# tim-speed/flexdiffuse

Hardware: AMD Instinct MI355X
Metric: 512x512 50-step images/sec/node (SD1.5, batch=8/GPU, Linear image guidance) (higher is better)
Workload: dtype fp16; 1 GPU; SD1.5 512x512 50-step DDIM + linear image guidance, CFG 8, batch=8/GPU (BASELINE configs[1]); parallelism=seed-sharded x1, preset=sd15, guidance=linear, img2img=False, unet_evaluations_per_image=50, launch=graph, scheduler=ddim

## Files before the change

### flexdiffuse_amd/csrc/common.h

```cpp
#pragma once
#include <hip/hip_runtime.h>
#include <stdint.h>
#include <stdio.h>
#include <string.h>

#include "../../include/flexdiffuse_hip.h"

void fd_set_error(const char* fmt, ...);

#define FD_CHECK_ARG(cond, code, ...)                  \
    do {                                               \
        if (!(cond)) {                                 \
            fd_set_error(__VA_ARGS__);                 \
            return (code);                             \
        }                                              \
    } while (0)

#define FD_CHECK_LAUNCH(name)                                                    \
    do {                                                                         \
        hipError_t e_ = hipGetLastError();                                       \
        if (e_ != hipSuccess) {                                                  \
            fd_set_error("%s: launch failed: %s", (name), hipGetErrorString(e_)); \
            return FD_EHIP;                                                      \
        }                                                                        \
    } while (0)

#define FD_HIP(call)                                                                 \
    do {                                                                             \
        hipError_t e_ = (call);                                                      \
        if (e_ != hipSuccess) {                                                      \
            fd_set_error("%s failed: %s", #call, hipGetErrorString(e_));             \
            return FD_EHIP;                                                          \
        }                                                                            \
    } while (0)

static inline int fd_cdiv(int a, int b) { return (a + b - 1) / b; }
static inline int fd_grid1d(size_t total, int cap) {
    const size_t blocks = (total + 255) / 256;
    return (int)(blocks < (size_t)cap ? blocks : (size_t)cap);
}

#ifdef __cplusplus
#include <functional>
bool fd_plan_recording();
void fd_plan_push(std::function<int(void*)> op);
#define FD_PLAN(...)                                                            \
    do {                                                                        \
        if (fd_plan_recording())                                                \
            fd_plan_push([=](void* fd_s_) -> int { return __VA_ARGS__; });      \
    } while (0)
#endif

void fd_prof_begin(int family, hipStream_t s, double work, double executed = -1.0, unsigned tag = 0);
void fd_prof_end(int family, hipStream_t s);
#ifdef __cplusplus
struct FdProfScope {
    int family;
    hipStream_t st;
    FdProfScope(int f, void* stream, double bytes, unsigned tag = 0) : family(f), st((hipStream_t)stream) { fd_prof_begin(f, st, bytes, -1.0, tag); }
    ~FdProfScope() { fd_prof_end(family, st); }
};
static inline unsigned fd_tag(unsigned a, unsigned b = 0, unsigned c = 0, unsigned d = 0, unsigned e = 0, unsigned f = 0) {
    unsigned h = 2166136261u;
    const unsigned v[6] = {a, b, c, d, e, f};
    for (int i = 0; i < 6; ++i) h = (h ^ v[i]) * 16777619u;
    return h | 1u;
}
#endif

#ifdef __cplusplus
#include <atomic>
static inline bool fd_first_on_device(std::atomic<unsigned long long>* mask) {
    int dev = 0;
    if (hipGetDevice(&dev) != hipSuccess) return true;
    const unsigned long long bit = 1ull << (dev & 63);
    return (mask->fetch_or(bit) & bit) == 0;
}
#endif

typedef _Float16 half_t;
typedef half_t half8 __attribute__((ext_vector_type(8)));
typedef half_t half4 __attribute__((ext_vector_type(4)));
typedef half_t half2v __attribute__((ext_vector_type(2)));
typedef float floatx2 __attribute__((ext_vector_type(2)));
typedef float floatx4 __attribute__((ext_vector_type(4)));
typedef float floatx16 __attribute__((ext_vector_type(16)));

__device__ __forceinline__ float fd_wave_sum(float v) {
#pragma unroll
    for (int o = 32; o > 0; o >>= 1) v += __shfl_xor(v, o, 64);
    return v;
}
__device__ __forceinline__ float fd_wave_max(float v) {
#pragma unroll
    for (int o = 32; o > 0; o >>= 1) v = fmaxf(v, __shfl_xor(v, o, 64));
    return v;
}
```

### flexdiffuse_amd/csrc/gemm.hip

```cpp
#include "gemm_epilogue.h"
#include "gn_slab.h"

typedef const __attribute__((address_space(1))) half_t* gptr_h;
typedef const __attribute__((address_space(1))) u32x4* gptr_u4;

template <int BM, int BN, bool TRANS, bool CONV>
__global__ __launch_bounds__(256) void k_gemm_f16(GemmArgs g) {
    constexpr int WTM = BM / 2, WTN = BN / 2;
    constexpr int MI = WTM / 16, NI = WTN / 16;
    constexpr int AR = BM / 32, BR = BN / 32;
    constexpr int STAGE = (BM + BN) * 128;
    extern __shared__ __attribute__((aligned(16))) char smem[];

    const int tid = threadIdx.x, lane = tid & 63, wave = tid >> 6;
    const int wm = wave >> 1, wn = wave & 1;

    const int nb = g.tiles_m * g.tiles_n;
    int id = blockIdx.x;
    {
        const int q = nb >> 3, r = nb & 7, xcd = id & 7, slot = id >> 3;
        id = (xcd < r ? xcd * (q + 1) : r * (q + 1) + (xcd - r) * q) + slot;
    }
    const int tile_n = id % g.tiles_n, tile_m = id / g.tiles_n;
    const int m0 = tile_m * BM, n0 = tile_n * BN;
// ... 694 lines not shown

template <int S>
__device__ __forceinline__ void splitk_finish_body(const GemmArgs& g) {
    const int n4 = g.N >> 2;
    const size_t total = (size_t)g.M * n4;
    const size_t slab = (size_t)g.M * g.N;
    for (size_t e = (size_t)blockIdx.x * 256 + threadIdx.x; e < total; e += (size_t)gridDim.x * 256) {
        const int m = (int)(e / n4), nb0 = (int)(e - (size_t)m * n4) * 4;
        const float* src = g.ws + (size_t)m * g.N + nb0;
        float4 p[S > 0 ? S : 1];
        if constexpr (S > 0) {
#pragma unroll
            for (int s = 0; s < S; ++s) p[s] = *reinterpret_cast<const float4*>(src + (size_t)s * slab);
        } else {
            p[0] = *reinterpret_cast<const float4*>(src);
        }
        float4 bb = make_float4(0.f, 0.f, 0.f, 0.f), b2 = bb;
        half4 rr = {(half_t)0.f, (half_t)0.f, (half_t)0.f, (half_t)0.f};
        if (g.bias) bb = *reinterpret_cast<const float4*>(g.bias + nb0);
        if (g.bias2) b2 = *reinterpret_cast<const float4*>(g.bias2 + (size_t)(m / g.rows_per_batch) * g.ldb2 + nb0);
        if (g.res) rr = *reinterpret_cast<const half4*>(g.res + (size_t)(g.res_rows ? m % g.res_rows : m) * g.ldr + nb0);
        float4 a = p[0];
        if constexpr (S > 0) {
#pragma unroll
            for (int s = 1; s < S; ++s) { a.x += p[s].x; a.y += p[s].y; a.z += p[s].z; a.w += p[s].w; }
        } else {
            for (int s = 1; s < g.split_k; ++s) {
                const float4 q = *reinterpret_cast<const float4*>(src + (size_t)s * slab);
                a.x += q.x; a.y += q.y; a.z += q.z; a.w += q.w;
            }
        }
        const float bs[4] = {bb.x + b2.x, bb.y + b2.y, bb.z + b2.z, bb.w + b2.w};
        float v[4] = {fmaf(a.x, g.alpha, bs[0]), fmaf(a.y, g.alpha, bs[1]), fmaf(a.z, g.alpha, bs[2]), fmaf(a.w, g.alpha, bs[3])};
#pragma unroll
        for (int r = 0; r < 4; ++r) v[r] = act_apply(v[r], g.act);
        if (g.res) {
#pragma unroll
            for (int r = 0; r < 4; ++r) v[r] += (float)rr[r];
        }
        if (g.out_f32) {
            *reinterpret_cast<float4*>(reinterpret_cast<float*>(g.C) + (size_t)m * g.ldc + nb0) =
                make_float4(v[0], v[1], v[2], v[3]);
        } else {
            half4 o;
#pragma unroll
            for (int r = 0; r < 4; ++r) o[r] = (half_t)v[r];
            *reinterpret_cast<half4*>(reinterpret_cast<half_t*>(g.C) + (size_t)m * g.ldc + nb0) = o;
        }
    }
}

__global__ __launch_bounds__(256) void k_splitk_finish(GemmArgs g) {
    switch (g.split_k) {
        case 2: splitk_finish_body<2>(g); break;
        case 4: splitk_finish_body<4>(g); break;
        case 8: splitk_finish_body<8>(g); break;
        case 16: splitk_finish_body<16>(g); break;
        default: splitk_finish_body<0>(g); break;
    }
}


template <int S>
__global__ __launch_bounds__(256) void k_splitk_finish_gn(GemmArgs g) {
    extern __shared__ float gn_sm[];
    constexpr int NT = 256, NV = 16;
    const int HW = g.rows_per_batch, C = g.N, cpg = C / g.gn_groups, GB = g.gn_gb, CB = cpg * GB, c8 = CB >> 3;
    const int b = blockIdx.x, ch0 = blockIdx.y * CB, tid = threadIdx.x;
    const int cc = tid % c8;
    const int n = ch0 + cc * 8;
    float bs[8];
#pragma unroll
    for (int k = 0; k < 8; ++k) bs[k] = 0.f;
    if (g.bias) {
        const float4 lo = *reinterpret_cast<const float4*>(g.bias + n), hi = *reinterpret_cast<const float4*>(g.bias + n + 4);
        bs[0] = lo.x; bs[1] = lo.y; bs[2] = lo.z; bs[3] = lo.w; bs[4] = hi.x; bs[5] = hi.y; bs[6] = hi.z; bs[7] = hi.w;
    }
    if (g.bias2) {
        const float* b2 = g.bias2 + (size_t)b * g.ldb2 + n;
        const float4 lo = *reinterpret_cast<const float4*>(b2), hi = *reinterpret_cast<const float4*>(b2 + 4);
        bs[0] += lo.x; bs[1] += lo.y; bs[2] += lo.z; bs[3] += lo.w; bs[4] += hi.x; bs[5] += hi.y; bs[6] += hi.z; bs[7] += hi.w;
    }
    const size_t slab = (size_t)g.M * g.N;
    const size_t row0 = (size_t)b * HW;
    const float* __restrict__ src0 = g.ws + row0 * g.N + n;
    const int PL = NT / c8, pl = tid / c8;
    const int nv = (HW + PL - 1) / PL;
    const bool active = pl < PL;
    constexpr int CH = S >= 16 ? 1 : (S >= 8 ? 2 : (S >= 4 ? 4 : 8));
    static_assert(NV % CH == 0, "whole chunks");
    auto fill = [&](uint4(&v)[NV]) __attribute__((always_inline)) {
#pragma unroll
        for (int i0 = 0; i0 < NV; i0 += CH) {
            if (i0 < nv) {
                float4 lo[CH][S], hi[CH][S];
                half8 rr[CH];
#pragma unroll
                for (int j = 0; j < CH; ++j) {
                    const int p = min(pl + PL * (i0 + j), HW - 1);
                    const float* src = src0 + (size_t)p * g.N;
#pragma unroll
                    for (int s = 0; s < S; ++s) {
                        lo[j][s] = *reinterpret_cast<const float4*>(src + (size_t)s * slab);
                        hi[j][s] = *reinterpret_cast<const float4*>(src + (size_t)s * slab + 4);
                    }
                }
                if (g.res) {
#pragma unroll
                    for (int j = 0; j < CH; ++j)
                        rr[j] = *reinterpret_cast<const half8*>(g.res + (row0 + min(pl + PL * (i0 + j), HW - 1)) * g.ldr + n);
                }
#pragma unroll
                for (int j = 0; j < CH; ++j) {
                    float a[8] = {lo[j][0].x, lo[j][0].y, lo[j][0].z, lo[j][0].w, hi[j][0].x, hi[j][0].y, hi[j][0].z, hi[j][0].w};
#pragma unroll
                    for (int s = 1; s < S; ++s) {
                        a[0] += lo[j][s].x; a[1] += lo[j][s].y; a[2] += lo[j][s].z; a[3] += lo[j][s].w;
                        a[4] += hi[j][s].x; a[5] += hi[j][s].y; a[6] += hi[j][s].z; a[7] += hi[j][s].w;
                    }
                    half8 o;
#pragma unroll
                    for (int k = 0; k < 8; ++k) {
                        float val = fmaf(a[k], g.alpha, bs[k]);
                        if (g.res) val += (float)rr[j][k];
                        o[k] = (half_t)val;
                    }
                    const int p = pl + PL * (i0 + j);
                    const bool valid = active && p < HW;
                    const uint4 packed = *reinterpret_cast<uint4*>(&o);
                    v[i0 + j] = valid ? packed : make_uint4(0u, 0u, 0u, 0u);
                }
            } else {
#pragma unroll
                for (int j = 0; j < CH; ++j) v[i0 + j] = make_uint4(0u, 0u, 0u, 0u);
            }
        }
        if (!g.gn_skip_c && active) {
            half_t* __restrict__ cb = reinterpret_cast<half_t*>(g.C) + row0 * g.ldc + n;
#pragma unroll
            for (int i = 0; i < NV; ++i) {
                const int p = pl + PL * i;
                if (p < HW) *reinterpret_cast<uint4*>(cb + (size_t)p * g.ldc) = v[i];
            }
        }
    };
    gn_slab_body<NT, NV>(fill, g.gn_out + row0 * C + ch0, g.gn_gamma + ch0, g.gn_beta + ch0, HW, C, cpg, GB, g.gn_eps, g.gn_silu, gn_sm);
}

template <int S>
static int launch_finish_gn(const GemmArgs& g, hipStream_t st) {
    size_t lds = 0;
    const int GB = gn_slab_pick<256, 16>(g.rows_per_batch, g.N, g.gn_groups, &lds);
    static std::atomic<unsigned long long> configured{0};
    if (lds > 64 * 1024 && fd_first_on_device(&configured))
        FD_HIP(hipFuncSetAttribute(reinterpret_cast<const void*>(k_splitk_finish_gn<S>), hipFuncAttributeMaxDynamicSharedMemorySize, 160 * 1024));
    hipLaunchKernelGGL(k_splitk_finish_gn<S>, dim3(g.M / g.rows_per_batch, g.gn_groups / GB), dim3(256), lds, st, g);
    FD_CHECK_LAUNCH("k_splitk_finish_gn");
    return FD_OK;
}

extern "C" int fd_gemm_can_fuse_groupnorm(int M, int N, int rows_per_sample, int groups, int split_k) {
    if (M <= 0 || N <= 0 || rows_per_sample <= 0 || groups <= 0 || M % rows_per_sample != 0 || N % 8 != 0 || N % groups != 0) return 0;
    if (!(split_k == 2 || split_k == 4 || split_k == 8 || split_k == 16)) return 0;
    size_t lds = 0;
    return gn_slab_pick<256, 16>(rows_per_sample, N, groups, &lds) > 0 ? 1 : 0;
}

static bool g_use_dma = getenv("FD_GEMM_NO_DMA") == nullptr;
static int g_tap_fast = getenv("FD_CONV_TAPFAST") ? atoi(getenv("FD_CONV_TAPFAST")) : 1;
static int g_pp = getenv("FD_GEMM_PP") ? atoi(getenv("FD_GEMM_PP")) : 1;
static int g_bias_lds = getenv("FD_GEMM_BIAS_LDS") ? atoi(getenv("FD_GEMM_BIAS_LDS")) : 1;
static int g_fast_epi = getenv("FD_GEMM_FAST_EPI") ? atoi(getenv("FD_GEMM_FAST_EPI")) : 1;
static int g_persist_mode = getenv("FD_GEMM_PERSIST") ? atoi(getenv("FD_GEMM_PERSIST")) : 1;

static bool gemm_lean_dma_path() { return g_use_dma && g_fast_epi && g_bias_lds; }

struct GemmExtents {
    unsigned long long a, w, c;
    static bool below_2gib(unsigned long long elems) { return 2 * elems < 0x7fffffffull; }
    bool dma_ok() const { return below_2gib(a) && below_2gib(w); }
};
static GemmExtents gemm_extents(const GemmArgs& g, bool conv) {
    const unsigned long long a = conv ? ((unsigned long long)(g.M / (g.Ho * g.Wo)) * g.Hi * g.Wi - 1) * g.Cpix + g.Cin : (unsigned long long)(g.M - 1) * g.lda + g.K;
    return {a, (unsigned long long)(g.N - 1) * g.ldw + g.K, (unsigned long long)(g.M - 1) * g.ldc + g.N};
}

template <int BM, int BN, bool TRANS, bool CONV, int WM = 2, int NS = 2, int WN = 2, int EPI = 0>
static int launch_mode(GemmArgs& g, int batch, hipStream_t st) {
    g.tiles_m = fd_cdiv(g.M, BM);
    g.tiles_n = fd_cdiv(g.N, BN);
    const size_t lds = NS * (size_t)(BM + BN) * 128 + 4 * BN * sizeof(float) + ((EPI == 5 || EPI == 6 || EPI == 7 || EPI == 13 || EPI == 14) ? BM * 2 * sizeof(float) : 0);
    dim3 grid(g.tiles_m * g.tiles_n, g.split_k, batch);
    const unsigned long long a_bytes =
        CONV ? 2ull * (((unsigned long long)(g.M / (g.Ho * g.Wo)) * g.Hi * g.Wi - 1) * g.Cpix + g.Cin)
             : 2ull * ((unsigned long long)(g.M - 1) * g.lda + g.K);
    const unsigned long long w_bytes = 2ull * ((unsigned long long)(g.N - 1) * g.ldw + g.K + g.K2);
    if (g_use_dma && a_bytes < 0x7fffffffull && w_bytes < 0x7fffffffull) {
        static std::atomic<unsigned long long> configured{0};
        if (lds > 64 * 1024 && fd_first_on_device(&configured)) {
            FD_HIP(hipFuncSetAttribute(reinterpret_cast<const void*>(k_gemm_f16_dma<BM, BN, CONV, WM, TRANS, NS, WN, EPI>),
                                       hipFuncAttributeMaxDynamicSharedMemorySize, (int)lds));
            if constexpr (BN != 320 && EPI != 13 && EPI != 14)
                FD_HIP(hipFuncSetAttribute(reinterpret_cast<const void*>(k_gemm_f16_dmap<BM, BN, CONV, WM, TRANS, WN, EPI>),
                                           hipFuncAttributeMaxDynamicSharedMemorySize, (int)lds));
        }
        const int occ = (BM >= 256 || lds > 80 * 1024) ? 1 : (BM * BN >= 128 * 128) ? 2 : (BM == 128 ? 3 : 4);
        const int slots = 256 * occ;
        const int nkt = (g.K + BK - 1) / BK / g.split_k;
        const bool persistent = NS == 2 && BN != 320 && EPI != 13 && g.K2 == 0 && !g.phase && !g.ln_stats_out && g.ln_parts <= 1 && g.strideBias == 0 && (g_persist_mode == 2 ||
                                (g_persist_mode == 1 && nkt <= 20 && g.tiles_m * g.tiles_n > slots));
        if constexpr (EPI >= 1 && EPI <= 3) {
            if (persistent && g.bias2) return launch_mode<BM, BN, TRANS, CONV, WM, NS, WN, 0>(g, batch, st);
        }
        if (persistent) {
            if constexpr (BN != 320 && EPI != 13 && EPI != 14) {
                dim3 pgrid(g.tiles_m * g.tiles_n > slots ? slots : g.tiles_m * g.tiles_n, g.split_k, batch);
                hipLaunchKernelGGL((k_gemm_f16_dmap<BM, BN, CONV, WM, TRANS, WN, EPI>), pgrid, dim3(64 * WM * WN), lds,
                                   st, g, (unsigned)a_bytes, (unsigned)w_bytes);
            }
        } else {
            hipLaunchKernelGGL((k_gemm_f16_dma<BM, BN, CONV, WM, TRANS, NS, WN, EPI>), grid, dim3(64 * WM * WN), lds, st, g,
                               (unsigned)a_bytes, (unsigned)w_bytes);
        }
        FD_CHECK_LAUNCH("k_gemm_f16_dma");
        return FD_OK;
    }
    if (g.ln_stats) {
        fd_set_error("fd_gemm_f16: the LayerNorm fold needs the LDS-DMA path (tensor < 2 GiB, FD_GEMM_NO_DMA unset)");
        return FD_ESHAPE;
    }
    if (g.K2) {
        fd_set_error("fd_gemm_f16: the appended 1x1 phase (A2 / K2) needs the LDS-DMA path (tensor < 2 GiB, FD_GEMM_NO_DMA unset)");
        return FD_ESHAPE;
    }
    if constexpr (EPI != 0) {
        return launch_mode<BM, BN, TRANS, CONV, WM, NS, WN, 0>(g, batch, st);
    } else if constexpr (WM != 2 || WN != 2) {
        fd_set_error("fd_gemm_f16: 8-wave tiles need the LDS-DMA path (tensor < 2 GiB)");
        return FD_ESHAPE;
    } else {
        static std::atomic<unsigned long long> configured{0};
        if (lds > 64 * 1024 && fd_first_on_device(&configured))
            FD_HIP(hipFuncSetAttribute(reinterpret_cast<const void*>(k_gemm_f16<BM, BN, TRANS, CONV>),
                                       hipFuncAttributeMaxDynamicSharedMemorySize, (int)lds));
        hipLaunchKernelGGL((k_gemm_f16<BM, BN, TRANS, CONV>), grid, dim3(256), lds, st, g);
        FD_CHECK_LAUNCH("k_gemm_f16");
        return FD_OK;
    }
}

template <int BM, int BN, bool TRANS, int WM = 2, int NS = 2, int WN = 2, int EPI = 0>
static int launch(GemmArgs& g, int batch, hipStream_t st) {
    return g.mode == MODE_CONV ? launch_mode<BM, BN, TRANS, true, WM, NS, WN, EPI>(g, batch, st)
                               : launch_mode<BM, BN, TRANS, false, WM, NS, WN, EPI>(g, batch, st);
}

template <int BM, int BN, int WM, int NS, int WN, int ALLOW>
static int launch_epi(GemmArgs& g, int batch, hipStream_t st) {
    const bool full = g_fast_epi && g.split_k == 1 && !g.out_f32 && !g.trans_out && g.bias_lds &&
                      g.M % BM == 0 && g.N % BN == 0 && (g.ldc & 7) == 0 &&
                      (!g.bias2 || g.rows_per_batch % BM == 0);
    if (g.gn_part_out) {
        if constexpr (BN == 320 && NS == 2) {
            if (full && g.act == FD_ACT_NONE && !g.ln_stats && !g.ln_stats_out && g.N == BN && g.rows_per_batch % BM == 0 && !g.phase && batch == 1 &&
                (!g.res || (g.ldr & 3) == 0)) {
                if (g.res) return launch<BM, BN, false, WM, NS, WN, 12>(g, batch, st);
                return launch<BM, BN, false, WM, NS, WN, 11>(g, batch, st);
            }
        }
        fd_set_error("fd_gemm_f16: gn_part_out needs full 320-wide tiles inside one sample and the lean plain / residual epilogue");
        return FD_ESHAPE;
    }
    if (g.ln_stats_out) {
        if constexpr ((ALLOW & 256) != 0) {
            if (full && (BN != 320 || g.N == BN) && g.act == FD_ACT_NONE && g.mode != MODE_CONV && !g.ln_stats && !g.bias2) {
                if (g.res && (g.ldr & 3) == 0) return launch_mode<BM, BN, false, false, WM, NS, WN, 9>(g, batch, st);
                if (!g.res) return launch_mode<BM, BN, false, false, WM, NS, WN, 8>(g, batch, st);
            }
        }
        fd_set_error("fd_gemm_f16: ln_stats_out needs full tiles of a tile shape with a statistics epilogue, a plain or residual linear GEMM");
        return FD_ESHAPE;
    }
    if (full && g.ln_stats) {
        if (g.mode != MODE_CONV && !g.res) {
            if constexpr ((ALLOW & 64) != 0 && (BN / WN / 16) % 2 == 0) {
                if (g.act == FD_ACT_GEGLU) return launch_mode<BM, BN, false, false, WM, NS, WN, 6>(g, batch, st);
            }
            if constexpr ((ALLOW & 32) != 0) {
                if (g.act == FD_ACT_NONE) return launch_mode<BM, BN, false, false, WM, NS, WN, 5>(g, batch, st);
            }
        }
        return launch_mode<128, 128, false, false, 2, 2, 2, 7>(g, batch, st);
    }
    if (g.ln_stats) return launch_mode<128, 128, false, false, 2, 2, 2, 7>(g, batch, st);
    if (full) {
        if constexpr ((ALLOW & 8) != 0 && (BN / WN / 16) % 2 == 0) {
            if (g.act == FD_ACT_GEGLU) return launch<BM, BN, false, WM, NS, WN, 3>(g, batch, st);
        }
        if constexpr ((ALLOW & 4) != 0) {
            if (g.act == FD_ACT_NONE && g.res && (g.ldr & 3) == 0) return launch<BM, BN, false, WM, NS, WN, 2>(g, batch, st);
        }
        if constexpr ((ALLOW & 2) != 0) {
            if (g.act == FD_ACT_NONE && !g.res) return launch<BM, BN, false, WM, NS, WN, 1>(g, batch, st);
        }
    }
    return launch<BM, BN, false, WM, NS, WN, 0>(g, batch, st);
}

#include "gemm_xfold.h"

static double fd_round_eff(long long tiles, int slots) {
    return (double)tiles / (double)((long long)slots * ((tiles + slots - 1) / slots));
}

static int fd_stats_plan(int M, int N, int* tile, int batch = 1) {
    if (N < 320 || N % 160 != 0) return 0;
    const bool ok23 = M % 288 == 0 && M >= 1152;
    if (N == 320 && M % 256 == 0) {
        if (ok23 && fd_round_eff((long long)(M / 288) * 2, 256) > fd_round_eff(M / 256, 256) + 0.08) {
            *tile = 23;
            return 2;
        }
        *tile = 16;
        return 1;
    }
    if (ok23 && (M % 128 != 0 ||
                 fd_round_eff((long long)(M / 288) * (N / 160), 256) >
                     (M % 256 == 0 && M > 4096 ? fd_round_eff((long long)(M / 256) * (N / 160), 256)
                                                : fd_round_eff((long long)(M / 128) * (N / 160), 512)) + 0.08)) {
        *tile = 23;
        return N / 160;
    }
    if (N != 320 && batch > 1 && M % 64 == 0 && M % 128 != 0) {
        *tile = 26;
        return N / 160;
    }
    if (N == 320 || M % 128 != 0) return 0;
    if (batch > 1 && M <= 256 && N >= 1280) {
        *tile = 20;
        return N / 160;
    }
    *tile = (M % 256 == 0 && (long long)M * batch > 4096) ? 13 : 12;
    return N / 160;
}

extern "C" int fd_gemm_can_emit_row_stats(int M, int N, int K, int ldc, int ldr) {
    if (!gemm_lean_dma_path()) return 0;
    if (M <= 0 || K <= 0 || K % 8 != 0) return 0;
    if (ldc < N || (ldc & 7) != 0 || (ldr != 0 && (ldr < N || (ldr & 3) != 0))) return 0;
    if (!GemmExtents::below_2gib((unsigned long long)(M - 1) * (unsigned long long)ldc + N)) return 0;
    int tile = 0;
    return fd_stats_plan(M, N, &tile);
}


struct GemmPlan {
    int tile, split, batch;
    int gn_parts_bm;
    double flops, flops_exec;
    unsigned tag;
};

enum { FORM_RULE, FORM_TRANS_TAIL, FORM_SOFTMAX, FORM_TRANS_OUT };
static int gemm_form(const GemmArgs& g) { return g.tr_n0 ? FORM_TRANS_TAIL : (g.sm_valid ? FORM_SOFTMAX : (g.trans_out ? FORM_TRANS_OUT : FORM_RULE)); }

static void gemm_tile_shape(int tile, int* bm, int* bn) {
    switch (tile) {
        case 9: case 12: case 20: *bm = 128; *bn = 160; break;
        case 10: *bm = 128; *bn = 128; break;
        case 13: *bm = 256; *bn = 160; break;
        case 14: *bm = 256; *bn = 128; break;
        case 15: *bm = 256; *bn = 256; break;
        case 16: *bm = 256; *bn = 320; break;
        case 23: *bm = 288; *bn = 160; break;
        case 26: *bm = 64; *bn = 160; break;
        default: fd_gemm_pp_tile_shape(tile, bm, bn); break;
    }
}

static bool gemm_tile_ln_fold(int tile) {
    return tile == 9 || tile == 10 || (tile >= 12 && tile <= 16) || tile == 20 || tile == 23 || tile == 26 || tile >= 30;
}

static bool gemm_pp_ok(GemmArgs g, int batch, int tile, int split) {
    g.split_k = split;
    return fd_gemm_pp_ok(g, batch, tile);
}

static int gemm_grow_split(const GemmArgs& g, size_t ws_bytes, long long tiles, int target, int cap, int min_kt) {
    if (!g.ws || g.N % 4 != 0) return 1;
    const int nk_all = (g.K + g.K2 + BK - 1) / BK;
    int split = 1;
    while (tiles * split < target && split < cap && nk_all / (split * 2) >= min_kt && (size_t)(split * 2) * g.M * g.N * 4 <= ws_bytes) split *= 2;
    return split;
}

static int gn_parts_bm(const GemmArgs& g, int tile, int split, int batch, int groups) {
// ... 448 lines not shown
```

### flexdiffuse_amd/csrc/gemm_pp.hip

```cpp
#include "gemm_epilogue.h"

typedef __attribute__((address_space(3))) void* lds_ptr;

template <int WM_, int WN_, int MI, int NI, bool CONV, int EPI, bool HAS_K2>
__global__ __launch_bounds__(512) void k_gemm_f16_pp(GemmArgs g, unsigned a_bytes, unsigned w_bytes) {
#if defined(__HIP_DEVICE_COMPILE__)
    static_assert(WM_ * WN_ == 8 && MI % 2 == 0, "8 waves; the row halves must be equal");
    constexpr int WTM = MI * 16, WTN = NI * 16, BM = WM_ * WTM, BN = WN_ * WTN;
    constexpr int MH = MI / 2, NI0 = (NI + 1) / 2, NI1 = NI / 2;
    constexpr int PA = WM_ * MH * 16, PB0 = WN_ * NI0 * 16, PB1 = WN_ * NI1 * 16;
    constexpr int OA0 = 0, OB0 = PA * 128, OB1 = OB0 + PB0 * 128, OA1 = OB1 + PB1 * 128, STAGE = OA1 + PA * 128;
    constexpr int GA = PA / 8, GB0 = PB0 / 8, GB1 = PB1 / 8;
    constexpr int CA = (GA + 7) / 8, CB0 = (GB0 + 7) / 8, CB1 = (GB1 + 7) / 8;
    static_assert(GA % 8 == 0 && GB1 % 8 == 0, "only B0 may leave some waves one DMA short");
    constexpr int INFLIGHT = 2 * (GA / 8) + GB0 / 8 + GB1 / 8;
    extern __shared__ __attribute__((aligned(16))) char smem[];

#ifdef FD_PP_STAMPS
    const unsigned long long ts_start = __builtin_amdgcn_s_memtime();
    const unsigned long long rt_start = __builtin_amdgcn_s_memrealtime();
    unsigned long long ts_a[4] = {0, 0, 0, 0}, ts_b[4] = {0, 0, 0, 0}, ts_d[4] = {0, 0, 0, 0};
#define PP_STAMP(X) X = __builtin_amdgcn_s_memtime();
#else
#define PP_STAMP(X)
// ... 249 lines not shown
    PP_BAR();
    const bool late = wave >= 4;
    if (late) { PP_BAR(); }
#ifdef FD_PP_STAMPS
    const unsigned long long ts_loop0 = __builtin_amdgcn_s_memtime();
#endif
    int l = 0;
#pragma clang loop unroll(disable)
    for (; l + 1 < nkl; l += 2) {
        PP_PHASE(0) PP_PHASE(1) PP_PHASE(2) PP_PHASE(3)
        PP_PHASE(4) PP_PHASE(5) PP_PHASE(6) PP_PHASE(7)
    }
#ifdef FD_PP_STAMPS
    const unsigned long long ts_sa[4] = {ts_a[0], ts_a[1], ts_a[2], ts_a[3]}, ts_sb[4] = {ts_b[0], ts_b[1], ts_b[2], ts_b[3]},
                             ts_sd[4] = {ts_d[0], ts_d[1], ts_d[2], ts_d[3]};
#endif
    if (l < nkl) {
        PP_PHASE(0) PP_PHASE(1) PP_PHASE(2) PP_PHASE(3)
    }
    if (!late) { PP_BAR(); }
#ifdef FD_PP_STAMPS
    const unsigned long long ts_loop1 = __builtin_amdgcn_s_memtime();
#endif
#undef PP_PHASE
#undef PP_WAIT
#undef PP_BAR
#undef PP_MFMA
#undef PP_READ_A
#undef PP_READ_B0
#undef PP_READ_B1
#undef PP_ISSUE
#undef PP_ISSUE_A
#undef PP_ISSUE_B
#undef PP_PREP
#undef PP_PREP_A
#undef PP_PREP_B
#undef PP_ADVANCE
#undef PP_GROUP_ROW
#undef PP_B_ROW
#undef PP_IS_A2
#undef PP_UNIFORM
#undef PP_FLAG

    if constexpr (EPI == 10) {
        float* __restrict__ P = g.ws + (size_t)kslice * g.M * g.N + (size_t)(m0 + wm * WTM + fr) * g.N + n0 + wn * WTN + fq * 4;
#pragma unroll
        for (int i = 0; i < MI; ++i)
#pragma unroll
            for (int j = 0; j < NI; ++j) {
#ifdef FD_SPLITK_NO_STORE
                asm volatile("" ::"v"(acc[i][j]));
                if (g.M < 0)
#endif
                *reinterpret_cast<floatx4*>(P + (size_t)i * 16 * g.N + j * 16) = acc[i][j];
            }
    } else if constexpr (EPI == 14) {
        {
            float* __restrict__ P = g.ws + (size_t)kslice * g.M * g.N + (size_t)(m0 + wm * WTM + fr) * g.N + n0 + wn * WTN + fq * 4;
#pragma unroll
            for (int i = 0; i < MI; ++i)
#pragma unroll
                for (int j = 0; j < NI; ++j) *reinterpret_cast<floatx4*>(P + (size_t)i * 16 * g.N + j * 16) = acc[i][j];
        }
        const int tile_id = tile_m * g.tiles_n + tile_n;
        unsigned* arrive = g.sk_sync + tile_id;
        unsigned* depart = g.sk_sync + g.tiles_m * g.tiles_n + tile_id;
        __syncthreads();
        if (tid == 0) {
            __hip_atomic_fetch_add(arrive, 1u, __ATOMIC_RELEASE, __HIP_MEMORY_SCOPE_AGENT);
            int spins = 0;
            while (__hip_atomic_load(arrive, __ATOMIC_ACQUIRE, __HIP_MEMORY_SCOPE_AGENT) < (unsigned)g.split_k && ++spins < (1 << 22))
                __builtin_amdgcn_s_sleep(4);
        }
        __syncthreads();
        {
            const int S = g.split_k, rows = BM / S, r0 = m0 + kslice * rows;
            constexpr int C4 = BN / 4;
            const size_t slab = (size_t)g.M * g.N;
            for (int e = tid; e < rows * C4; e += 512) {
                const int r = e / C4, c4 = e - r * C4;
                const int m = r0 + r, n = n0 + c4 * 4;
                const float* src = g.ws + (size_t)m * g.N + n;
                float4 a = *reinterpret_cast<const float4*>(src);
                for (int sidx = 1; sidx < S; ++sidx) {
                    const float4 q = *reinterpret_cast<const float4*>(src + (size_t)sidx * slab);
                    a.x += q.x; a.y += q.y; a.z += q.z; a.w += q.w;
                }
                float4 bb = make_float4(0.f, 0.f, 0.f, 0.f), b2 = bb;
                if (g.bias) bb = *reinterpret_cast<const float4*>(g.bias + n);
                if (g.bias2) b2 = *reinterpret_cast<const float4*>(g.bias2 + (size_t)(m / g.rows_per_batch) * g.ldb2 + n);
                float v[4] = {fmaf(a.x, g.alpha, bb.x + b2.x), fmaf(a.y, g.alpha, bb.y + b2.y), fmaf(a.z, g.alpha, bb.z + b2.z), fmaf(a.w, g.alpha, bb.w + b2.w)};
                if (g.res) {
                    const half4 rr = *reinterpret_cast<const half4*>(g.res + (size_t)(g.res_rows ? m % g.res_rows : m) * g.ldr + n);
#pragma unroll
                    for (int k = 0; k < 4; ++k) v[k] += (float)rr[k];
                }
                half4 o;
#pragma unroll
                for (int k = 0; k < 4; ++k) o[k] = (half_t)v[k];
                *reinterpret_cast<half4*>(reinterpret_cast<half_t*>(g.C) + (size_t)m * g.ldc + n) = o;
            }
        }
        __syncthreads();
        if (tid == 0) {
            const unsigned old = __hip_atomic_fetch_add(depart, 1u, __ATOMIC_RELAXED, __HIP_MEMORY_SCOPE_AGENT);
            if (old == (unsigned)g.split_k - 1u) {
                __hip_atomic_store(arrive, 0u, __ATOMIC_RELAXED, __HIP_MEMORY_SCOPE_AGENT);
                __hip_atomic_store(depart, 0u, __ATOMIC_RELAXED, __HIP_MEMORY_SCOPE_AGENT);
            }
        }
    } else if constexpr (EPI == 0 || EPI == 7)
        gemm_epilogue<BM, BN, false, WM_, WN_, EPI == 7>(g, acc, m0, n0, wm, wn, fr, fq, z, (g.bias && g.bias_lds) ? (lds_cfloat)bias_s : (lds_cfloat) nullptr,
                                                         b2_staged ? (lds_cfloat)(bias_s + BN) : (lds_cfloat) nullptr, kslice, stats_tile);
    else if constexpr (EPI == 8 || EPI == 9) {
        asm volatile("s_waitcnt vmcnt(0)" ::: "memory");
        __syncthreads();
        gemm_epilogue_fast<MI, NI, FD_ACT_NONE, EPI == 9, true, false, true, WN_>(
            g, acc, m0 + wm * WTM + fr, n0 + wn * WTN, wn * WTN, fq, z, (lds_cfloat)bias_s, (lds_cfloat)(bias_s + BN),
            reinterpret_cast<float*>(smem), wm * WTM + fr, wn, m0);
    } else if constexpr (EPI == 11 || EPI == 12) {
        asm volatile("s_waitcnt vmcnt(0)" ::: "memory");
        __syncthreads();
        gemm_epilogue_fast<MI, NI, FD_ACT_NONE, EPI == 12, true, false, false, WN_, WM_>(
            g, acc, m0 + wm * WTM + fr, n0 + wn * WTN, wn * WTN, fq, z, (lds_cfloat)bias_s, (lds_cfloat)(bias_s + BN),
            reinterpret_cast<float*>(smem), wm * WTM + fr, wn, m0);
    } else
        gemm_epilogue_fast<MI, NI, (EPI == 3 || EPI == 6) ? FD_ACT_GEGLU : FD_ACT_NONE, EPI == 2, true, (EPI == 5 || EPI == 6)>(
            g, acc, m0 + wm * WTM + fr, n0 + wn * WTN, wn * WTN, fq, z, (lds_cfloat)bias_s, (lds_cfloat)(bias_s + BN),
            nullptr, wm * WTM + fr, wn, m0, stats_tile);
#ifdef FD_PP_STAMPS
    if (EPI != 10 && g.ws && lane == 0) {
        unsigned long long* o = reinterpret_cast<unsigned long long*>(g.ws) + ((size_t)blockIdx.x * 8 + wave) * 16;
        o[0] = ts_start; o[1] = ts_loop0; o[2] = ts_loop1; o[3] = __builtin_amdgcn_s_memtime();
#pragma unroll
        for (int p = 0; p < 3; ++p) { o[4 + 3 * p] = ts_sa[p]; o[5 + 3 * p] = ts_sb[p]; o[6 + 3 * p] = ts_sd[p]; }
        o[13] = ts_sa[3]; o[14] = ts_sb[3];
        o[15] = __builtin_amdgcn_s_memrealtime() - rt_start;
    }
#endif
#undef PP_STAMP
#endif
}

template <int WM_, int WN_, int MI, int NI, bool CONV, int EPI, bool HAS_K2>
static int pp_launch_k2(GemmArgs& g, int batch, hipStream_t st) {
    constexpr int BM = WM_ * MI * 16, BN = WN_ * NI * 16;
    g.tiles_m = g.M / BM;
    g.tiles_n = g.N / BN;
    const size_t lds = 2 * (size_t)(BM + BN) * 128 + 4 * BN * sizeof(float) + ((EPI == 5 || EPI == 6 || EPI == 7) ? BM * 2 * sizeof(float) : 0);
    const unsigned long long a_bytes = CONV ? 2ull * (((unsigned long long)(g.M / (g.Ho * g.Wo)) * g.Hi * g.Wi - 1) * g.Cpix + g.Cin)
                                            : 2ull * ((unsigned long long)(g.M - 1) * g.lda + g.K);
    const unsigned long long w_bytes = 2ull * ((unsigned long long)(g.N - 1) * g.ldw + g.K + g.K2);
    static std::atomic<unsigned long long> configured{0};
    if (fd_first_on_device(&configured))
        FD_HIP(hipFuncSetAttribute(reinterpret_cast<const void*>(k_gemm_f16_pp<WM_, WN_, MI, NI, CONV, EPI, HAS_K2>),
                                   hipFuncAttributeMaxDynamicSharedMemorySize, (int)lds));
    static const int sk_xcd = getenv("FD_PP_SK_XCD") ? atoi(getenv("FD_PP_SK_XCD")) : 1;
    const int nb = g.tiles_m * g.tiles_n;
    g.sk_flat = sk_xcd && (g.split_k == 2 || g.split_k == 4 || g.split_k == 8) && batch == 1 && nb % (8 / g.split_k) == 0 &&
                (nb * g.split_k) % 8 == 0;
    const dim3 grid = g.sk_flat ? dim3(nb * g.split_k, 1, batch) : dim3(nb, g.split_k, batch);
    hipLaunchKernelGGL((k_gemm_f16_pp<WM_, WN_, MI, NI, CONV, EPI, HAS_K2>), grid, dim3(512), lds, st, g,
                       (unsigned)a_bytes, (unsigned)w_bytes);
    FD_CHECK_LAUNCH("k_gemm_f16_pp");
    return FD_OK;
}

template <int WM_, int WN_, int MI, int NI, bool CONV, int EPI>
static int pp_launch_k(GemmArgs& g, int batch, hipStream_t st) {
    if constexpr (EPI == 1 || EPI == 2 || EPI == 10 || EPI == 0 || EPI == 11 || EPI == 12 || EPI == 14) {
        if (g.K2) return pp_launch_k2<WM_, WN_, MI, NI, CONV, EPI, true>(g, batch, st);
    } else {
        if (g.K2) {
            fd_set_error("fd_gemm_f16: the appended A2 phase has no ping-pong kernel with this epilogue");
            return FD_ESHAPE;
        }
    }
    return pp_launch_k2<WM_, WN_, MI, NI, CONV, EPI, false>(g, batch, st);
}

template <int WM_, int WN_, int MI, int NI>
static int pp_launch(GemmArgs& g, int batch, hipStream_t st) {
    constexpr int BM = WM_ * MI * 16, BN = WN_ * NI * 16;
    const bool conv = g.mode == MODE_CONV;
    if (g.split_k > 1 && (g.N & 3) == 0 && g.sk_sync) {
        if constexpr (BN == 320) {
            if ((g.M / BM) * (g.N / BN) * g.split_k <= 256 && BM % g.split_k == 0 && batch == 1 && !g.out_f32 && g.act == FD_ACT_NONE && (g.ldc & 3) == 0 &&
                (!g.res || (g.ldr & 3) == 0) && (g.ldb2 & 3) == 0)
                return conv ? pp_launch_k<WM_, WN_, MI, NI, true, 14>(g, batch, st) : pp_launch_k<WM_, WN_, MI, NI, false, 14>(g, batch, st);
        }
        fd_set_error("fd_gemm_f16: sk_sync (in-launch split-K reduction) needs a 320-wide ping-pong tile, tiles x split_k <= 256 workgroups, a plain fp16 output");
        return FD_ESHAPE;
    }
    if (g.split_k > 1 && (g.N & 3) == 0)
        return conv ? pp_launch_k<WM_, WN_, MI, NI, true, 10>(g, batch, st) : pp_launch_k<WM_, WN_, MI, NI, false, 10>(g, batch, st);
    const bool lean = g.split_k == 1 && !g.out_f32 && !g.trans_out && g.bias_lds && (g.ldc & 7) == 0 &&
                      (!g.bias2 || g.ln_stats || g.rows_per_batch % BM == 0);
    if (g.gn_part_out) {
        if constexpr (BN == 320) {
            if (lean && g.act == FD_ACT_NONE && !g.ln_stats && !g.ln_stats_out && g.N == BN && g.rows_per_batch % BM == 0 && !g.phase && batch == 1 &&
                (!g.res || (g.ldr & 3) == 0)) {
                if (g.res) return conv ? pp_launch_k<WM_, WN_, MI, NI, true, 12>(g, batch, st) : pp_launch_k<WM_, WN_, MI, NI, false, 12>(g, batch, st);
                return conv ? pp_launch_k<WM_, WN_, MI, NI, true, 11>(g, batch, st) : pp_launch_k<WM_, WN_, MI, NI, false, 11>(g, batch, st);
            }
        }
        fd_set_error("fd_gemm_f16: gn_part_out on a ping-pong tile needs the lean epilogue of a 320-wide tile inside one sample");
        return FD_ESHAPE;
    }
    if (g.ln_stats_out) {
        if (lean && !conv && (WN_ == 2 || g.N == BN) && g.act == FD_ACT_NONE && !g.ln_stats && !g.bias2) {
            if (g.res && (g.ldr & 3) == 0) return pp_launch_k<WM_, WN_, MI, NI, false, 9>(g, batch, st);
            if (!g.res) return pp_launch_k<WM_, WN_, MI, NI, false, 8>(g, batch, st);
        }
        fd_set_error("fd_gemm_f16: ln_stats_out on a ping-pong tile needs the lean epilogue of a plain or residual linear GEMM");
        return FD_ESHAPE;
    }
    if (g.ln_stats) {
        if (lean && !conv && !g.res) {
            if constexpr (NI % 2 == 0) {
                if (g.act == FD_ACT_GEGLU) return pp_launch_k<WM_, WN_, MI, NI, false, 6>(g, batch, st);
            }
            if (g.act == FD_ACT_NONE) return pp_launch_k<WM_, WN_, MI, NI, false, 5>(g, batch, st);
        }
        if (!conv) return pp_launch_k<WM_, WN_, MI, NI, false, 7>(g, batch, st);
        fd_set_error("fd_gemm_f16: LayerNorm fold on a convolution");
        return FD_ESHAPE;
    }
    if (lean) {
        if constexpr (NI % 2 == 0) {
            if (g.act == FD_ACT_GEGLU && !conv) return pp_launch_k<WM_, WN_, MI, NI, false, 3>(g, batch, st);
        }
        if (g.act == FD_ACT_NONE && g.res && (g.ldr & 3) == 0)
            return conv ? pp_launch_k<WM_, WN_, MI, NI, true, 2>(g, batch, st) : pp_launch_k<WM_, WN_, MI, NI, false, 2>(g, batch, st);
        if (g.act == FD_ACT_NONE && !g.res)
            return conv ? pp_launch_k<WM_, WN_, MI, NI, true, 1>(g, batch, st) : pp_launch_k<WM_, WN_, MI, NI, false, 1>(g, batch, st);
    }
    return conv ? pp_launch_k<WM_, WN_, MI, NI, true, 0>(g, batch, st) : pp_launch_k<WM_, WN_, MI, NI, false, 0>(g, batch, st);
}

void fd_gemm_pp_tile_shape(int tile, int* bm, int* bn) {
    switch (tile) {
        case 30: *bm = 256; *bn = 320; break;
        case 31: *bm = 256; *bn = 256; break;
        case 32: *bm = 128; *bn = 320; break;
        case 33: *bm = 256; *bn = 160; break;
        default: *bm = *bn = 0; break;
    }
}

bool fd_gemm_pp_ok(const GemmArgs& g, int batch, int tile) {
    int bm, bn;
    fd_gemm_pp_tile_shape(tile, &bm, &bn);
    if (!bm) return false;
    if (g.M % bm != 0 || g.N % bn != 0 || g.K % BK != 0 || g.K2 % BK != 0 || g.trans_out) return false;
    if (g.act == FD_ACT_GEGLU && (bn / (tile == 33 ? 2 : 4)) % 32 != 0) return false;
    const unsigned long long a_bytes = g.mode == MODE_CONV ? 2ull * (((unsigned long long)(g.M / (g.Ho * g.Wo)) * g.Hi * g.Wi - 1) * g.Cpix + g.Cin)
                                                           : 2ull * ((unsigned long long)(g.M - 1) * g.lda + g.K);
    const unsigned long long w_bytes = 2ull * ((unsigned long long)(g.N - 1) * g.ldw + g.K + g.K2);
    if (a_bytes >= 0x7ffffff0ull || w_bytes >= 0x7ffffff0ull) return false;
    if (g.mode == MODE_CONV) {
        if (g.Wo % 8 != 0 || g.up || g.Cin % BK != 0) return false;
        if (g.K2 && (g.stride != 1 || g.Ho != g.Hi || g.Wo != g.Wi || g.phase)) return false;
    }
    if (g.split_k > 1 && (g.K / BK + g.K2 / BK) / g.split_k < 2) return false;
    (void)batch;
    return true;
}

int fd_gemm_pp_launch(GemmArgs& g, int batch, hipStream_t st, int tile) {
    switch (tile) {
        case 30: return pp_launch<2, 4, 8, 5>(g, batch, st);
        case 31: return pp_launch<2, 4, 8, 4>(g, batch, st);
        case 32: return pp_launch<2, 4, 4, 5>(g, batch, st);
        case 33: return pp_launch<4, 2, 4, 5>(g, batch, st);
        default: fd_set_error("fd_gemm_f16: unknown ping-pong tile %d", tile); return FD_EINVAL;
    }
}
```

### flexdiffuse_amd/csrc/norm.hip

```cpp
#include <stdlib.h>

#include "common.h"
#include "gn_slab.h"

#define GN_MAX_CHUNKS 256

__global__ void k_gn_stats(const half_t* __restrict__ x, float* __restrict__ part, int HW, int C,
                           int G, int PL, int pix_per_chunk, int ldx) {
    extern __shared__ float sm[];
    const int b = blockIdx.y, chunk = blockIdx.x;
    const int c8 = C >> 3;
    const int tid = threadIdx.x;
    const int cc = tid % c8, pl = tid / c8;
    const int p0 = chunk * pix_per_chunk;
    const int p1 = min(HW, p0 + pix_per_chunk);
    float s[8], q[8];
#pragma unroll
    for (int k = 0; k < 8; ++k) s[k] = q[k] = 0.f;
    if (pl < PL) {
        const half_t* base = x + ((size_t)b * HW) * ldx + cc * 8;
        int p = p0 + pl;
        uint4 raw[4], nxt[4];
        bool have = p + 3 * PL < p1;
        if (have) {
// ... 59 lines not shown
            bq += sm[(size_t)(g * cpg + i) * 2 + 1];
        }
        a = fd_wave_sum(a);
        bq = fd_wave_sum(bq);
        if (lane == 0) {
            float* dst = part + (((size_t)b * gridDim.x + chunk) * G + g) * 2;
            dst[0] = a;
            dst[1] = bq;
        }
    }
}

__global__ void k_gn_apply(const half_t* __restrict__ x, half_t* __restrict__ y,
                           const float* __restrict__ part, const float* __restrict__ gamma,
                           const float* __restrict__ beta, int HW, int C, int G,
                           int nchunk_stats, int PL, int pix_per_chunk, float eps, int silu, int ldx) {
    extern __shared__ float sm[];
    const int b = blockIdx.y, chunk = blockIdx.x, tid = threadIdx.x;
    const int nt = blockDim.x, nsub = nt / G;
    double* red = reinterpret_cast<double*>(sm);
    float* gst = reinterpret_cast<float*>(red + 2 * nsub * G);
    {
        const int g = tid % G, sub = tid / G;
        if (sub < nsub) {
            double s = 0.0, q = 0.0;
            const float2* src = reinterpret_cast<const float2*>(part) + ((size_t)b * nchunk_stats) * G + g;
            int k = sub;
            for (; k + 3 * nsub < nchunk_stats; k += 4 * nsub) {
                float2 v[4];
#pragma unroll
                for (int u = 0; u < 4; ++u) v[u] = src[(size_t)(k + u * nsub) * G];
#pragma unroll
                for (int u = 0; u < 4; ++u) {
                    s += (double)v[u].x;
                    q += (double)v[u].y;
                }
            }
            for (; k < nchunk_stats; k += nsub) {
                const float2 v = src[(size_t)k * G];
                s += (double)v.x;
                q += (double)v.y;
            }
            red[sub * G + g] = s;
            red[nsub * G + sub * G + g] = q;
        }
    }
    __syncthreads();
    const int cpg = C / G;
    if (tid < G) {
        double s = 0.0, q = 0.0;
        for (int u = 0; u < nsub; ++u) {
            s += red[u * G + tid];
            q += red[nsub * G + u * G + tid];
        }
        const double n = (double)HW * cpg;
        const double mean = s / n;
        double var = q / n - mean * mean;
        if (var < 0.0) var = 0.0;
        gst[tid * 2 + 0] = (float)mean;
        gst[tid * 2 + 1] = (float)(1.0 / sqrt(var + (double)eps));
    }
    __syncthreads();
    const int c8 = C >> 3;
    const int cc = tid % c8, pl = tid / c8;
    if (pl >= PL) return;
    float sc[8], sh[8];
#pragma unroll
    for (int k = 0; k < 8; ++k) {
        const int c = cc * 8 + k, g = c / cpg;
        const float a = gst[g * 2 + 1] * gamma[c];
        sc[k] = a;
        sh[k] = beta[c] - gst[g * 2 + 0] * a;
    }
    const int p0 = chunk * pix_per_chunk;
    const int p1 = min(HW, p0 + pix_per_chunk);
    const half_t* xb = x + ((size_t)b * HW) * ldx + cc * 8;
    half_t* yb = y + ((size_t)b * HW) * C + cc * 8;
    int p = p0 + pl;
    uint4 raw[4], nxt[4];
    bool have = p + 3 * PL < p1;
    if (have) {
#pragma unroll
        for (int u = 0; u < 4; ++u) raw[u] = *reinterpret_cast<const uint4*>(xb + (size_t)(p + u * PL) * ldx);
    }
    while (have) {
        const int pn = p + 4 * PL;
        const bool more = pn + 3 * PL < p1;
        if (more) {
#pragma unroll
            for (int u = 0; u < 4; ++u) nxt[u] = *reinterpret_cast<const uint4*>(xb + (size_t)(pn + u * PL) * ldx);
        }
#pragma unroll
        for (int u = 0; u < 4; ++u) {
            const half8 v = *reinterpret_cast<const half8*>(&raw[u]);
            half8 o;
#pragma unroll
            for (int k = 0; k < 8; ++k) o[k] = (half_t)gn_act(fmaf((float)v[k], sc[k], sh[k]), silu);
            *reinterpret_cast<uint4*>(yb + (size_t)(p + u * PL) * C) = *reinterpret_cast<uint4*>(&o);
        }
#pragma unroll
        for (int u = 0; u < 4; ++u) raw[u] = nxt[u];
        p = pn;
        have = more;
    }
    for (; p < p1; p += PL) {
        const uint4 raw = *reinterpret_cast<const uint4*>(xb + (size_t)p * ldx);
        const half8 v = *reinterpret_cast<const half8*>(&raw);
        half8 o;
#pragma unroll
        for (int k = 0; k < 8; ++k) o[k] = (half_t)gn_act(fmaf((float)v[k], sc[k], sh[k]), silu);
        *reinterpret_cast<uint4*>(yb + (size_t)p * C) = *reinterpret_cast<uint4*>(&o);
    }
}

template <int NT, int NV>
__global__ __launch_bounds__(NT) void k_gn_slab(const half_t* __restrict__ x, half_t* __restrict__ y,
                                                const float* __restrict__ gamma,
                                                const float* __restrict__ beta, int HW, int C,
                                                int G, int GB, float eps, int silu, int ldx) {
    extern __shared__ float sm[];
    const int cpg = C / G, CB = cpg * GB, c8 = CB >> 3;
    const int PL = NT / c8;
    const int b = blockIdx.x, ch0 = blockIdx.y * CB, tid = threadIdx.x;
    const int cc = tid % c8, pl = tid / c8;
    const half_t* xb = x + (size_t)b * HW * ldx + ch0;
    const unsigned xoff0 = (unsigned)(pl * ldx + cc * 8), xstep = (unsigned)(PL * ldx);
    const bool active = pl < PL;
    gn_slab_body<NT, NV>(
        [&](uint4(&v)[NV]) __attribute__((always_inline)) {
#pragma unroll
            for (int i = 0; i < NV; ++i) {
                const int p = pl + PL * i;
                v[i] = make_uint4(0u, 0u, 0u, 0u);
                if (active && p < HW) v[i] = *reinterpret_cast<const uint4*>(xb + (xoff0 + xstep * i));
            }
        },
        y + (size_t)b * HW * C + ch0, gamma + ch0, beta + ch0, HW, C, cpg, GB, eps, silu, sm);
}

template <int NT, int NV>
static bool gn_try_slab(const void* x, void* y, const float* gamma, const float* beta, int B,
                        int HW, int C, int G, float eps, int silu, hipStream_t st, int* rc, int ldx) {
    size_t lds = 0;
    const int GB = gn_slab_pick<NT, NV>(HW, C, G, &lds);
    if (!GB) return false;
    static std::atomic<unsigned long long> attr_set{0};
    if (fd_first_on_device(&attr_set)) {
        if (hipFuncSetAttribute(reinterpret_cast<const void*>(k_gn_slab<NT, NV>),
                                hipFuncAttributeMaxDynamicSharedMemorySize, 160 * 1024) != hipSuccess) {
            fd_set_error("fd_groupnorm_nhwc_f16: cannot raise the LDS limit");
            *rc = FD_EHIP;
            return true;
        }
    }
    fd_prof_begin(FD_FAMILY_GROUPNORM, st, (double)B * HW * C * 4.0, -1.0, fd_tag(7u, B, HW, C, NT));
    hipLaunchKernelGGL((k_gn_slab<NT, NV>), dim3(B, G / GB), dim3(NT), lds, st, (const half_t*)x,
                       (half_t*)y, gamma, beta, HW, C, G, GB, eps, silu, ldx);
    fd_prof_end(FD_FAMILY_GROUPNORM, st);
    *rc = hipGetLastError() == hipSuccess ? FD_OK : FD_EHIP;
    if (*rc != FD_OK) fd_set_error("k_gn_slab: launch failed");
    return true;
}

#define GNF_ROWS 16
__global__ __launch_bounds__(256) void k_gn_fold_linear(const float* __restrict__ part, int nchunk_stats, int HW, int C, int G, float eps,
                                                        const half_t* __restrict__ wg,
                                                        const float* __restrict__ biasf, int N, half_t* __restrict__ w_out,
                                                        float* __restrict__ bias_out) {
    __shared__ float rstd_s[64], mean_s[64];
    __shared__ float gsum_s[GNF_ROWS][64];
    __shared__ double red_s[2][256];
    extern __shared__ __align__(16) unsigned char gnf_lds[];
    half_t* wr = reinterpret_cast<half_t*>(gnf_lds);
    const int b = blockIdx.y, tid = threadIdx.x;
    const int nsub = 256 / G;
    {
        const int g = tid % G, sub = tid / G;
        if (sub < nsub) {
            double s = 0.0, q = 0.0;
            const float2* src = reinterpret_cast<const float2*>(part) + ((size_t)b * nchunk_stats) * G + g;
            for (int k = sub; k < nchunk_stats; k += nsub) {
                const float2 v = src[(size_t)k * G];
                s += (double)v.x;
                q += (double)v.y;
            }
            red_s[0][sub * G + g] = s;
            red_s[1][sub * G + g] = q;
        }
    }
    __syncthreads();
    if (tid < G) {
        double s = 0.0, q = 0.0;
        for (int u = 0; u < nsub; ++u) {
            s += red_s[0][u * G + tid];
            q += red_s[1][u * G + tid];
        }
        const double n = (double)HW * (C / G);
        const double mean = s / n;
        double var = q / n - mean * mean;
        if (var < 0.0) var = 0.0;
        const double rstd = 1.0 / sqrt(var + (double)eps);
        rstd_s[tid] = (float)rstd;
        mean_s[tid] = (float)mean;
    }
    __syncthreads();
    const int n0 = blockIdx.x * GNF_ROWS, rows = min(GNF_ROWS, N - n0);
    const int c8 = C >> 3, cpg = C / G;
    for (int i = tid; i < rows * c8; i += 256) {
        const int r = i / c8, cc = i - r * c8;
        const half8 v = *reinterpret_cast<const half8*>(wg + (size_t)(n0 + r) * C + cc * 8);
        half8 o;
#pragma unroll
        for (int k = 0; k < 8; ++k) o[k] = (half_t)((float)v[k] * rstd_s[(cc * 8 + k) / cpg]);
        *reinterpret_cast<half8*>(w_out + ((size_t)b * N + n0 + r) * C + cc * 8) = o;
        *reinterpret_cast<half8*>(wr + (size_t)r * C + cc * 8) = o;
    }
    __syncthreads();
    for (int i = tid; i < rows * G; i += 256) {
        const int r = i / G, g = i - r * G;
        const half_t* src = wr + (size_t)r * C + g * cpg;
        float acc = 0.f;
        for (int c = 0; c < cpg; ++c) acc += (float)src[c];
        gsum_s[r][g] = acc;
    }
    __syncthreads();
    if (tid < rows) {
        float acc = biasf[n0 + tid];
        for (int g = 0; g < G; ++g) acc = fmaf(-mean_s[g], gsum_s[tid][g], acc);
        bias_out[(size_t)b * N + n0 + tid] = acc;
    }
}

static void gn_stats_shape(int B, int HW, int C, int* PL, int* threads, int* nchunk, int* ppc) {
    const int c8 = C / 8;
    int pl = 512 / c8;
    if (pl < 1) pl = 1;
    if (pl > HW) pl = HW;
    int nc = 256 / B;
    if (nc < 1) nc = 1;
    if (nc > GN_MAX_CHUNKS) nc = GN_MAX_CHUNKS;
    int pp = fd_cdiv(HW, nc);
    if (pp < pl) pp = pl;
    *PL = pl;
    *threads = ((c8 * pl + 63) / 64) * 64;
    *ppc = pp;
    *nchunk = fd_cdiv(HW, pp);
}

extern "C" int fd_groupnorm_fold_linear_f16(const void* x, int ldx, float* ws, int B, int HW, int C, int G, float eps,
                                            const void* wg, const float* biasf, int N,
                                            void* w_out, float* bias_out, void* stream) {
    FD_PLAN(fd_groupnorm_fold_linear_f16(x, ldx, ws, B, HW, C, G, eps, wg, biasf, N, w_out, bias_out, fd_s_));
    FD_CHECK_ARG(x && ws && wg && biasf && w_out && bias_out, FD_EINVAL, "fd_groupnorm_fold_linear_f16: null pointer");
    FD_CHECK_ARG(B > 0 && HW > 0 && C > 0 && G > 0 && N > 0, FD_EINVAL, "fd_groupnorm_fold_linear_f16: bad dims");
    FD_CHECK_ARG(C % 8 == 0 && C % G == 0 && G <= 64 && C / 8 <= 1024, FD_ESHAPE,
                 "fd_groupnorm_fold_linear_f16: C=%d must be a multiple of 8 and of G=%d (G <= 64)", C, G);
    FD_CHECK_ARG(ldx >= C && ldx % 8 == 0 && ((uintptr_t)x | (uintptr_t)wg | (uintptr_t)w_out) % 16 == 0, FD_ESHAPE,
                 "fd_groupnorm_fold_linear_f16: ldx=%d must be >= C=%d, a multiple of 8; x / wg / w_out 16-byte aligned", ldx, C);
    FD_CHECK_ARG((long long)B * HW * ldx < 0x7fffffffLL, FD_ESHAPE, "fd_groupnorm_fold_linear_f16: tensor too large");
    hipStream_t st = (hipStream_t)stream;
    int PL, threads, nchunk, ppc;
    gn_stats_shape(B, HW, C, &PL, &threads, &nchunk, &ppc);
    const size_t lds1 = (size_t)PL * C * 2 * sizeof(float);
    FD_CHECK_ARG(lds1 <= 64 * 1024, FD_ESHAPE, "fd_groupnorm_fold_linear_f16: stats LDS too large");
    const size_t lds2 = (size_t)GNF_ROWS * C * sizeof(half_t);
    FD_CHECK_ARG(lds2 <= 48 * 1024, FD_ESHAPE, "fd_groupnorm_fold_linear_f16: C=%d too wide for the fold kernel's weight tile", C);
    fd_prof_begin(FD_FAMILY_GROUPNORM, st, (double)B * HW * C * 2.0, -1.0, fd_tag(8u, B, HW, C, N));
    hipLaunchKernelGGL(k_gn_stats, dim3(nchunk, B), dim3(threads), lds1, st, (const half_t*)x, ws, HW, C, G, PL, ppc, ldx);
    hipLaunchKernelGGL(k_gn_fold_linear, dim3(fd_cdiv(N, GNF_ROWS), B), dim3(256), lds2, st, (const float*)ws, nchunk, HW, C, G, eps,
                       (const half_t*)wg, biasf, N, (half_t*)w_out, bias_out);
    fd_prof_end(FD_FAMILY_GROUPNORM, st);
    FD_CHECK_LAUNCH("k_gn_stats/k_gn_fold_linear");
    return FD_OK;
}

extern "C" int fd_groupnorm_fold_linear_parts_f16(const float* parts, int chunks, int B, int HW, int C, int G, float eps,
                                                  const void* wg, const float* biasf, int N, void* w_out, float* bias_out, void* stream) {
    FD_PLAN(fd_groupnorm_fold_linear_parts_f16(parts, chunks, B, HW, C, G, eps, wg, biasf, N, w_out, bias_out, fd_s_));
    FD_CHECK_ARG(parts && wg && biasf && w_out && bias_out, FD_EINVAL, "fd_groupnorm_fold_linear_parts_f16: null pointer");
    FD_CHECK_ARG(B > 0 && HW > 0 && C > 0 && G > 0 && N > 0 && chunks > 0, FD_EINVAL, "fd_groupnorm_fold_linear_parts_f16: bad dims");
    FD_CHECK_ARG(C % 8 == 0 && C % G == 0 && G <= 64 && ((uintptr_t)wg | (uintptr_t)w_out) % 16 == 0, FD_ESHAPE,
                 "fd_groupnorm_fold_linear_parts_f16: C=%d must be a multiple of 8 and of G=%d (G <= 64); wg / w_out 16-byte aligned", C, G);
    const size_t lds2 = (size_t)GNF_ROWS * C * sizeof(half_t);
    FD_CHECK_ARG(lds2 <= 48 * 1024, FD_ESHAPE, "fd_groupnorm_fold_linear_parts_f16: C=%d too wide for the fold kernel's weight tile", C);
    hipStream_t st = (hipStream_t)stream;
    fd_prof_begin(FD_FAMILY_GROUPNORM, st, 0.0, -1.0, fd_tag(12u, B, HW, C, N));
    hipLaunchKernelGGL(k_gn_fold_linear, dim3(fd_cdiv(N, GNF_ROWS), B), dim3(256), lds2, st, parts, chunks, HW, C, G, eps,
                       (const half_t*)wg, biasf, N, (half_t*)w_out, bias_out);
    fd_prof_end(FD_FAMILY_GROUPNORM, st);
    FD_CHECK_LAUNCH("k_gn_fold_linear");
    return FD_OK;
}

extern "C" int64_t fd_groupnorm_workspace_floats(int B, int G) {
    return (int64_t)B * GN_MAX_CHUNKS * G * 2;
}

extern "C" int fd_groupnorm_nhwc_f16(const void* x, void* y, const float* gamma,
                                     const float* beta, float* ws, int B, int HW, int C, int G,
                                     float eps, int silu, void* stream) {
    return fd_groupnorm_nhwc_ld_f16(x, C, y, gamma, beta, ws, B, HW, C, G, eps, silu, stream);
}

extern "C" int fd_groupnorm_nhwc_ld_f16(const void* x, int ldx, void* y, const float* gamma,
                                        const float* beta, float* ws, int B, int HW, int C, int G,
                                        float eps, int silu, void* stream) {
// ... 283 lines not shown
```

### flexdiffuse_amd/csrc/xattn.hip

```cpp
#include <stdlib.h>

#include "common.h"

#define XBK 64
typedef unsigned int xu32x2 __attribute__((ext_vector_type(2)));
typedef unsigned int xu32x4 __attribute__((ext_vector_type(4)));
typedef const __attribute__((address_space(3))) float* xlds_cfloat;
typedef const __attribute__((address_space(3))) floatx4* xlds_cf4;

struct XattnArgs {
    const half_t* A;
    const half_t* W;
    const float* bias;
    const float* colsum;
    const float* ln_stats;
    const char* kimg;
    const char* vimg;
    half_t* O;
    int M, lda, ldw, ldo;
    int rows_per_sample, samples_per_rep, n_keys;
    int ln_parts;
    float ln_inv_n, ln_eps;
};

// ... 222 lines not shown
#pragma unroll
            for (int j = 0; j < NI; ++j) {
                if (j + 1 < NI) fb[j + 1] = *reinterpret_cast<const half8*>(st + frag_b + (j + 1) * 2048 + sw);
#pragma unroll
                for (int i = 0; i < MI; ++i) acc[i][j] = __builtin_amdgcn_mfma_f32_16x16x32_f16(fb[j], fa[i], acc[i][j], 0, 0, 0);
                __builtin_amdgcn_sched_barrier(0);
            }
        }
        asm volatile("s_waitcnt vmcnt(0)" ::: "memory");
        __syncthreads();
        cur ^= 1;
    }
    const char* sK = smem + cur * STAGE;
    const char* sV = smem + (cur ^ 1) * STAGE;
    XA_DMA_IMAGE(rsVi, VIMG, cur ^ 1);

    half8 q0[MI], q1[MI], qT[MI];
    {
        floatx2 st[MI];
#pragma unroll
        for (int i = 0; i < MI; ++i)
            st[i] = *reinterpret_cast<const __attribute__((address_space(3))) floatx2*>(
                (xlds_cfloat)stats_s + 2 * (wm * WTM + i * 16 + fr));
#pragma unroll
        for (int j = 0; j < NI; ++j) {
            const floatx4 bb = *reinterpret_cast<xlds_cf4>((xlds_cfloat)bias_s + wn * WTN + j * 16 + fq * 4);
            const floatx4 cs = *reinterpret_cast<xlds_cf4>((xlds_cfloat)bias_s + BN + wn * WTN + j * 16 + fq * 4);
            constexpr int JT = D == 40 ? 2 : 4;
#pragma unroll
            for (int i = 0; i < MI; ++i)
#pragma unroll
                for (int r = 0; r < 4; ++r) {
                    const half_t q = (half_t)fmaf(acc[i][j][r], st[i][0], fmaf(st[i][1], cs[r], bb[r]));
                    if (j == JT) { qT[i][r] = q; qT[i][4 + r] = (half_t)0.f; }
                    else {
                        const int jj = j < JT ? j : j - 1;
                        if (jj == 0) q0[i][r] = q;
                        if (jj == 1) q0[i][4 + r] = q;
                        if (jj == 2) q1[i][r] = q;
                        if (jj == 3) q1[i][4 + r] = q;
                    }
                }
            __builtin_amdgcn_sched_barrier(0);
        }
    }
    const int kb_last_valid = g.n_keys - 64 - fq * 4;
    const __amdgpu_buffer_rsrc_t rsO = __builtin_amdgcn_make_buffer_rsrc((void*)g.O, 0, o_bytes, 0x00020000);
    const unsigned o_lane = (unsigned)(((m0 + wm * WTM + fr) * g.ldo + n0 + wn * WTN + fq * 4) * 2);
    const unsigned o_rep = (unsigned)rep * (unsigned)g.M * (unsigned)g.ldo * 2u;
    bool v_ready = false;
#pragma unroll
    for (int hh = 0; hh < cfg::HPW; ++hh) {
        const char* kh = sK + (wn * cfg::HPW + hh) * KHEAD;
        const char* vh = sV + (wn * cfg::HPW + hh) * VHEAD;
#pragma unroll
        for (int ip = 0; ip < MI / 2; ++ip) {
            floatx4 s[2][XA_KB];
#pragma unroll
            for (int kb = 0; kb < XA_KB; ++kb) {
                const half8 ka = *reinterpret_cast<const half8*>(kh + kb * KBB + lane * 16);
                half8 kbf = ka;
                if constexpr (D == 80) kbf = *reinterpret_cast<const half8*>(kh + kb * KBB + 1024 + lane * 16);
                const half4 k16 = *reinterpret_cast<const half4*>(kh + kb * KBB + cfg::KSF * 1024 + lane * 8);
                const half_t z = (half_t)0.f;
                const half8 k16x = {k16[0], k16[1], k16[2], k16[3], z, z, z, z};
#pragma unroll
                for (int t = 0; t < 2; ++t) {
                    const int i = ip * 2 + t;
                    floatx4 v;
                    if constexpr (D == 40) {
                        v = __builtin_amdgcn_mfma_f32_16x16x32_f16(ka, hh ? q1[i] : q0[i], floatx4{0.f, 0.f, 0.f, 0.f}, 0, 0, 0);
                    } else {
                        v = __builtin_amdgcn_mfma_f32_16x16x32_f16(ka, q0[i], floatx4{0.f, 0.f, 0.f, 0.f}, 0, 0, 0);
                        v = __builtin_amdgcn_mfma_f32_16x16x32_f16(kbf, q1[i], v, 0, 0, 0);
                    }
                    s[t][kb] = __builtin_amdgcn_mfma_f32_16x16x32_f16(k16x, qT[i], v, 0, 0, 0);
                }
            }
            half8 pk[2][3];
            float lsum[2] = {0.f, 0.f};
#pragma unroll
            for (int t = 0; t < 2; ++t) {
#pragma unroll
                for (int r = 0; r < 4; ++r)
                    if (r >= kb_last_valid) s[t][4][r] = -INFINITY;
                float mx = fmaxf(fmaxf(s[t][0][0], s[t][0][1]), fmaxf(s[t][0][2], s[t][0][3]));
#pragma unroll
                for (int kb = 1; kb < XA_KB; ++kb)
                    mx = fmaxf(mx, fmaxf(fmaxf(s[t][kb][0], s[t][kb][1]), fmaxf(s[t][kb][2], s[t][kb][3])));
                mx = fmaxf(mx, __shfl_xor(mx, 16, 64));
                mx = fmaxf(mx, __shfl_xor(mx, 32, 64));
#pragma unroll
                for (int kb = 0; kb < XA_KB; ++kb)
#pragma unroll
                    for (int r = 0; r < 4; ++r) {
                        const half_t ph = (half_t)__builtin_amdgcn_exp2f(s[t][kb][r] - mx);
                        pk[t][kb >> 1][(kb & 1) * 4 + r] = ph;
                        if constexpr (!cfg::ONES) lsum[t] += (float)ph;
                    }
#pragma unroll
                for (int r = 0; r < 4; ++r) pk[t][2][4 + r] = (half_t)0.f;
                if constexpr (!cfg::ONES) {
                    lsum[t] += __shfl_xor(lsum[t], 16, 64);
                    lsum[t] += __shfl_xor(lsum[t], 32, 64);
                }
            }
            if (!v_ready) {
                asm volatile("s_waitcnt vmcnt(0)" ::: "memory");
                __syncthreads();
                v_ready = true;
            }
            floatx4 o[2][cfg::DT];
#pragma unroll
            for (int dt = 0; dt < cfg::DT; ++dt) {
                const half8 v0 = *reinterpret_cast<const half8*>(vh + dt * 2560 + lane * 16);
                const half8 v1 = *reinterpret_cast<const half8*>(vh + dt * 2560 + 1024 + lane * 16);
                const half4 v2 = *reinterpret_cast<const half4*>(vh + dt * 2560 + 2048 + lane * 8);
                const half_t z = (half_t)0.f;
                const half8 v2x = {v2[0], v2[1], v2[2], v2[3], z, z, z, z};
#pragma unroll
                for (int t = 0; t < 2; ++t) {
                    floatx4 a = __builtin_amdgcn_mfma_f32_16x16x32_f16(v0, pk[t][0], floatx4{0.f, 0.f, 0.f, 0.f}, 0, 0, 0);
                    a = __builtin_amdgcn_mfma_f32_16x16x32_f16(v1, pk[t][1], a, 0, 0, 0);
                    o[t][dt] = __builtin_amdgcn_mfma_f32_16x16x32_f16(v2x, pk[t][2], a, 0, 0, 0);
                }
            }
#pragma unroll
            for (int t = 0; t < 2; ++t) {
                float l = lsum[t];
                if constexpr (cfg::ONES) l = __shfl(o[t][2][0], 32 + fr, 64);
                const float inv = __builtin_amdgcn_rcpf(l);
                const unsigned off = o_lane + (unsigned)(((ip * 2 + t) * 16 * g.ldo + hh * D) * 2);
#pragma unroll
                for (int dt = 0; dt < cfg::DT; ++dt) {
                    half4 v;
#pragma unroll
                    for (int r = 0; r < 4; ++r) v[r] = (half_t)(o[t][dt][r] * inv);
                    const unsigned vo = (D == 40 && dt == 2 && fq >= 2) ? 0xffffff00u : off + dt * 32;
                    __builtin_amdgcn_raw_buffer_store_b64(__builtin_bit_cast(xu32x2, v), rsO, vo, o_rep, 0);
                }
            }
        }
    }
#undef XA_DMA_TILE
#undef XA_DMA_IMAGE
#endif
}

template <int D>
static int xa_launch(const XattnArgs& g, int n_rep, unsigned a_bytes, unsigned w_bytes, unsigned o_bytes, hipStream_t st) {
    typedef XaCfg<D> cfg;
    constexpr size_t lds = 2 * (size_t)(cfg::BM + 320) * 128 + (2 * 320 + 2 * cfg::BM) * sizeof(float);
    static std::atomic<unsigned long long> configured{0};
    if (fd_first_on_device(&configured))
        FD_HIP(hipFuncSetAttribute(reinterpret_cast<const void*>(k_xattn<D>), hipFuncAttributeMaxDynamicSharedMemorySize, (int)lds));
    hipLaunchKernelGGL(k_xattn<D>, dim3(g.M / cfg::BM, n_rep, cfg::C / 320), dim3(1024), lds, st, g, a_bytes, w_bytes, o_bytes);
    return FD_OK;
}

extern "C" int fd_xattn_q_f16(const fd_xattn_desc* d, void* stream) {
    if (fd_plan_recording() && d) {
        const fd_xattn_desc dc_ = *d;
        fd_plan_push([dc_](void* fd_s_) -> int { return fd_xattn_q_f16(&dc_, fd_s_); });
    }
    FD_CHECK_ARG(d && d->x && d->wq && d->bias && d->ln_colsum && d->ln_stats && d->k_image && d->v_image && d->out,
                 FD_EINVAL, "fd_xattn_q_f16: null pointer");
    FD_CHECK_ARG(xa_supported(d->heads, d->head_dim), FD_ESHAPE,
                 "fd_xattn_q_f16: 8 heads x 40 or 8 x 80 only (got %d x %d)", d->heads, d->head_dim);
    const int C = d->heads * d->head_dim, bm = d->head_dim == 40 ? 256 : 128;
    FD_CHECK_ARG(d->M > 0 && d->M % bm == 0 && d->rows_per_sample > 0 && d->rows_per_sample % bm == 0 &&
                     d->M % d->rows_per_sample == 0,
                 FD_ESHAPE, "fd_xattn_q_f16: M=%d and rows_per_sample=%d must be multiples of %d", d->M, d->rows_per_sample, bm);
    FD_CHECK_ARG(d->n_keys > 64 && d->n_keys <= 80 && d->n_rep >= 1, FD_ESHAPE, "fd_xattn_q_f16: 65..80 keys, n_rep >= 1 (got %d keys)", d->n_keys);
    FD_CHECK_ARG(d->ldx % 8 == 0 && d->ldw % 8 == 0 && d->ldo % 4 == 0 && d->ldx >= C && d->ldw >= C && d->ldo >= C,
                 FD_ESHAPE, "fd_xattn_q_f16: leading dimensions");
    FD_CHECK_ARG((((uintptr_t)d->x | (uintptr_t)d->wq | (uintptr_t)d->k_image | (uintptr_t)d->v_image | (uintptr_t)d->bias |
                   (uintptr_t)d->ln_colsum | (uintptr_t)d->ln_stats) % 16 == 0) && (uintptr_t)d->out % 8 == 0,
                 FD_ESHAPE, "fd_xattn_q_f16: pointers must be 16-byte aligned");
    const unsigned long long a_bytes = 2ull * ((unsigned long long)(d->M - 1) * d->ldx + C);
    const unsigned long long w_bytes = 2ull * ((unsigned long long)(C - 1) * d->ldw + C);
    const unsigned long long o_bytes = 2ull * ((unsigned long long)((long long)d->n_rep * d->M - 1) * d->ldo + C);
    FD_CHECK_ARG(a_bytes < 0x7fffffffull && o_bytes < 0x7fffffffull, FD_ESHAPE, "fd_xattn_q_f16: tensor >= 2 GiB");
    XattnArgs g;
    g.A = (const half_t*)d->x; g.W = (const half_t*)d->wq; g.bias = d->bias; g.colsum = d->ln_colsum;
    g.ln_stats = d->ln_stats; g.kimg = (const char*)d->k_image; g.vimg = (const char*)d->v_image;
    g.O = (half_t*)d->out;
    g.M = d->M; g.lda = d->ldx; g.ldw = d->ldw; g.ldo = d->ldo;
    g.rows_per_sample = d->rows_per_sample;
    g.samples_per_rep = d->M / d->rows_per_sample; g.n_keys = d->n_keys;
    FD_CHECK_ARG(d->ln_stats_parts == 0 || d->ln_stats_parts == 2 || d->ln_stats_parts == 4 || d->ln_stats_parts == 8, FD_ESHAPE,
                 "fd_xattn_q_f16: ln_stats_parts=%d (0, 2, 4 or 8)", d->ln_stats_parts);
    g.ln_parts = d->ln_stats_parts; g.ln_inv_n = 1.0f / (float)C; g.ln_eps = d->ln_fold_eps > 0.f ? d->ln_fold_eps : 1e-5f;
    hipStream_t st = (hipStream_t)stream;
    const double flops = 2.0 * d->M * (double)C * C + 4.0 * (double)d->n_rep * d->M * d->n_keys * C;
    fd_prof_begin(FD_FAMILY_ATTENTION, st, flops, -1.0, fd_tag(5u, d->M, d->n_rep, d->head_dim, d->n_keys));
    const int rc = d->head_dim == 40 ? xa_launch<40>(g, d->n_rep, (unsigned)a_bytes, (unsigned)w_bytes, (unsigned)o_bytes, st)
                                     : xa_launch<80>(g, d->n_rep, (unsigned)a_bytes, (unsigned)w_bytes, (unsigned)o_bytes, st);
    fd_prof_end(FD_FAMILY_ATTENTION, st);
    if (rc != FD_OK) return rc;
    FD_CHECK_LAUNCH("k_xattn");
    return FD_OK;
}
```

### flexdiffuse_amd/hip.py

```python
from __future__ import annotations

import ctypes
import os
from ctypes import c_char_p, c_double, c_float, c_int, c_int32, c_int64, c_uint64, c_void_p
from typing import Optional

import torch

_HERE = os.path.dirname(os.path.abspath(__file__))
LIB_PATH = os.environ.get('FD_LIB_PATH') or os.path.join(_HERE, 'libflexdiffuse_hip.so')

FD_OK, FD_EINVAL, FD_ESHAPE, FD_EHIP = 0, -1, -2, -3


class FDError(RuntimeError):
    '''HIP runtime failure reported by libflexdiffuse_hip.so (FD_EHIP).'''


class fd_tween_params(ctypes.Structure):
    _fields_ = [('threshold_floor', c_double), ('threshold_mult', c_double),
                ('clustered', c_double), ('max_guidance', c_double),
                ('header_max', c_double), ('order', c_int32), ('reuse', c_int32)]


P = c_void_p
_SIGNATURES = {
    'fd_abi_version': (c_int, []),
    'fd_last_error': (c_char_p, []),
    'fd_device_info': (c_int, [c_int, P, P, P, P, c_int]),
    'fd_prof_enable': (c_int, [c_int]),
    'fd_prof_set_stride': (c_int, [c_int]),
    'fd_prof_collect': (c_int, [c_int, P, P, P]),
    'fd_prof_collect2': (c_int, [c_int, P, P, P, P]),
    'fd_prof_calibrate': (c_int, [c_int, P, P]),
    'fd_prof_drain': (c_int, [P, P, P, P, P, c_int64, P]),
    'fd_guidance_workspace_floats': (c_int64, [c_int, c_int, c_int]),
    'fd_guidance_map': (c_int, [P, P, P, P, P, c_int, c_int, c_int, c_int, c_int, c_int, c_int, P]),
    'fd_guidance_tween': (c_int, [P, P, P, P, P, P, P, P, P, c_int, c_int, c_int, c_int, c_int,
                                  ctypes.POINTER(fd_tween_params), P]),
    'fd_guidance_concept_override': (c_int, [P, P, P, P, P, c_int, c_int, c_int, P]),
    'fd_guidance_header_pull': (c_int, [P, P, c_int, c_int, c_int, P]),
    'fd_gemm_f16': (c_int, [P, P]),
    'fd_gemm_can_emit_row_stats': (c_int, [c_int, c_int, c_int, c_int, c_int]),
    'fd_gemm_plan': (c_int, [c_void_p, c_void_p, c_void_p]),
    'fd_gemm_can_fuse_groupnorm': (c_int, [c_int, c_int, c_int, c_int, c_int]),
    'fd_gemm_gn_parts_chunks': (c_int, [P]),
    'fd_groupnorm_apply_parts_f16': (c_int, [P, c_int, P, P, P, P, c_int, c_int, c_int, c_int, c_int, c_float, c_int, P]),
    'fd_groupnorm_fold_linear_parts_f16': (c_int, [P, c_int, c_int, c_int, c_int, c_int, c_float, P, P, c_int, P, P, P]),
    'fd_attention_f16': (c_int, [P, P]),
    'fd_xattn_image_bytes': (c_int64, [c_int, c_int]),
    'fd_xattn_pack_kv_f16': (c_int, [P, P, P, P, c_int, c_int, c_int, c_int, c_int, c_int, c_int64, c_int64, P]),
    'fd_xattn_q_f16': (c_int, [P, P]),
    'fd_groupnorm_workspace_floats': (c_int64, [c_int, c_int]),
    'fd_groupnorm_nhwc_f16': (c_int, [P, P, P, P, P, c_int, c_int, c_int, c_int, c_float, c_int, P]),
    'fd_groupnorm_nhwc_ld_f16': (c_int, [P, c_int, P, P, P, P, c_int, c_int, c_int, c_int, c_float, c_int, P]),
    'fd_layernorm_f16': (c_int, [P, P, P, P, c_int, c_int, c_int, c_int, c_float, c_int, P]),
    'fd_ln_row_stats_f16': (c_int, [P, P, c_int, c_int, c_int, c_float, P]),
    'fd_ln_finalize_stats_f32': (c_int, [P, P, c_int, c_int, c_int, c_float, P]),
    'fd_groupnorm_fold_linear_f16': (c_int, [P, c_int, P, c_int, c_int, c_int, c_int, c_float, P, P, c_int, P, P, P]),
    'fd_softmax_rows_f16': (c_int, [P, c_int, c_int, c_int, c_float, P]),
    'fd_nchw_f32_to_nhwc_f16': (c_int, [P, P, c_int, c_int, c_int, c_int, c_int, c_float, P]),
    'fd_nhwc_f32_to_nchw_f32': (c_int, [P, P, c_int, c_int, c_int, c_int, c_float, c_float, c_int, P]),
    'fd_im2col_f16': (c_int, [P, P] + [c_int] * 12 + [P]),
    'fd_conv3x3_narrow_f16': (c_int, [P, P, P, P, c_int, P, c_int, c_int, c_int, c_int, c_int, c_int, c_int, c_float, P]),
    'fd_concat_channels_f16': (c_int, [P, P, P, c_int64, c_int, c_int, P]),
    'fd_cfg_ddim_step_f32': (c_int, [P, P, P, c_int, c_int, c_int, c_int, c_int, c_float, c_float,
                                     c_float, c_float, c_float, c_int, c_int, P]),
    'fd_axpby_f32': (c_int, [P, P, P, c_int64, c_float, c_float, c_int, P]),
    'fd_embed_tokens_f16': (c_int, [P, P, P, P, c_int, c_int, c_int, c_int, P]),
    'fd_vit_assemble_f16': (c_int, [P, P, P, P, c_int, c_int, c_int, P]),
    'fd_timestep_embedding_f16': (c_int, [P, c_int, P, c_int, c_int, P]),
    'fd_copy2d_f16': (c_int, [P, c_int, P, c_int, c_int64, c_int, P]),
    'fd_repeat_rows_f16': (c_int, [P, c_int, P, c_int, c_int64, c_int, c_int, P]),
    'fd_plan_create': (c_int, [P]),
    'fd_plan_destroy': (c_int, [P]),
    'fd_plan_record_begin': (c_int, [P]),
    'fd_plan_record_end': (c_int, [P]),
    'fd_plan_size': (c_int, [P, P]),
    'fd_plan_replay': (c_int, [P, P]),
    'fd_region_blend_f32': (c_int, [P, P] + [c_int] * 7 + [c_float, P]),
    'fd_composite_step_f32': (c_int, [P, P, P, P, c_int, c_int, c_int, c_int, c_int, c_int, c_float, c_float,
                                      c_float, c_float, c_float, c_int, c_int, P]),
    'fd_cfg_ddim_masked_step_f32': (c_int, [P, P, P, P, P, c_int, c_int, c_int, c_int, c_int, c_float, c_float,
                                            c_float, c_float, c_float, c_int, c_float, c_float, P]),
    'fd_cfg_multistep_step_f32': (c_int, [P, P, P, P, P, P, P, c_int, c_int, c_int, c_int, c_int, c_float, c_float,
                                          c_float, c_float, c_float, c_float, c_float, c_float, P]),
    'fd_cfg_linear_multistep_step_f32': (c_int, [P, P, c_int, c_int] + [P] * 10 + [c_int] * 5 + [c_float] * 11 + [P]),
    'fd_philox_normal_f32': (c_int, [P, c_int64, c_int, c_uint64, c_int64, c_int, c_int, P]),
    'fd_cfg_ddim_noise_step_f32': (c_int, [P, P, P, P, P, c_int, c_int, c_int, c_int, c_int, c_float, c_float,
                                           c_float, c_float, c_float, c_int, c_float, c_float, c_float, c_uint64, c_int64,
                                           c_int, c_int, P]),
    'fd_cfg_multistep_noise_step_f32': (c_int, [P, P, P, P, P, P, P, c_int, c_int, c_int, c_int, c_int, c_float, c_float,
                                                c_float, c_float, c_float, c_float, c_float, c_float, c_float, c_uint64,
                                                c_int64, c_int, c_int, P]),
    'fd_cfg_rescale_ddim_step_f32': (c_int, [P, P, P, P, P, P, P, c_int, c_int, c_int, c_int, c_float, c_float, c_float,
                                             c_float, c_float, c_float, c_int, c_int, c_float, c_float, c_float, c_uint64,
                                             c_int64, c_int, P]),
    'fd_cfg_rescale_multistep_step_f32': (c_int, [P, P, P, P, P, P, P, P, c_int, c_int, c_int, c_int, c_float, c_float,
                                                  c_float, c_float, c_float, c_float, c_float, c_float, c_float, c_float,
                                                  c_uint64, c_int64, c_int, P]),
    'fd_composite_ddim_step_f32': (c_int, [P, P, P, c_int, P, P, P, P] + [c_int] * 5 + [c_float] * 5 + [c_int]
                                   + [c_float] * 3 + [c_uint64, c_int64, c_int, c_int, P]),
    'fd_composite_multistep_step_f32': (c_int, [P, P, P, c_int, P, P, P, P, P] + [c_int] * 5 + [c_float] * 9
                                        + [c_uint64, c_int64, c_int, c_int, P]),
    'fd_composite_linear_multistep_step_f32': (c_int, [P, P, P, c_int, c_int, c_int] + [P] * 10 + [c_int] * 5
                                               + [c_float] * 11 + [P]),
    'fd_lerp_f16': (c_int, [P, P, P, c_int64, c_float, P]),
    'fd_xattn_fold_rows_f32': (c_int, [P, P, P, P, c_int, c_int, c_int, c_int, c_int, c_int, P]),
    'fd_window_gather_f32': (c_int, [P, P] + [c_int] * 10 + [P]),
    'fd_window_step_f32': (c_int, [P, P, P, P] + [c_int] * 13 + [c_float] * 5 + [c_int, c_int, P]),
    'fd_window_ddim_step_f32': (c_int, [P] * 7 + [c_int] * 13 + [c_float] * 5 + [c_int] + [c_float] * 3
                                + [c_uint64, c_int64, c_int, P]),
    'fd_window_multistep_step_f32': (c_int, [P] * 8 + [c_int] * 13 + [c_float] * 9 + [c_uint64, c_int64, c_int, P]),
    'fd_cast_f32_to_f16': (c_int, [P, P, c_int64, P]),
    'fd_cast_f16_to_f32': (c_int, [P, P, c_int64, P]),
}

ABI_VERSION = 12
_lib: Optional[ctypes.CDLL] = None


def declared_symbols():
    return sorted(_SIGNATURES)


def lib() -> ctypes.CDLL:
    global _lib
    if _lib is None:
        if not os.path.exists(LIB_PATH):
            raise RuntimeError(
                f'{LIB_PATH} is missing: the HIP extension has not been built. Run '
                '`python -c "import __graft_entry__ as g; g.build()"` (or `make -C '
                'flexdiffuse_amd/csrc`). flexdiffuse_amd has no CPU fallback.')
        handle = ctypes.CDLL(LIB_PATH)
        for name, (res, args) in _SIGNATURES.items():
            fn = getattr(handle, name)
            fn.restype = res
            fn.argtypes = args
        if handle.fd_abi_version() != ABI_VERSION:
            raise RuntimeError('libflexdiffuse_hip.so ABI version mismatch; rebuild')
        _lib = handle
    return _lib


def check(rc: int, what: str = ''):
    if rc == FD_OK:
        return
    msg = lib().fd_last_error().decode('utf-8', 'replace')
    if rc in (FD_EINVAL, FD_ESHAPE):
        raise ValueError(f'{what}: {msg}')
    raise FDError(f'{what}: {msg} (code {rc})')


def call(name: str, *args):
    check(getattr(lib(), name)(*args), name)


def require_device(*tensors):
    for t in tensors:
        if t is not None and not t.is_cuda:
            raise RuntimeError('flexdiffuse_amd runs on an MI355X HIP device only; got a '
                               f'{t.device} tensor (there is no CPU fallback)')


def ptr(t: Optional[torch.Tensor]) -> c_void_p:
    if t is None:
        return c_void_p(0)
    return c_void_p(t.data_ptr())


_raw_stream = getattr(torch._C, '_cuda_getCurrentRawStream', None)
_raw_device = getattr(torch._C, '_cuda_getDevice', None)


def stream() -> c_void_p:
    if _raw_stream is not None and _raw_device is not None:
        return c_void_p(_raw_stream(_raw_device()))
    return c_void_p(torch.cuda.current_stream().cuda_stream)


def device_info(device: int = 0) -> dict:
    cu, khz, mem = c_int(0), c_int(0), c_int64(0)
    arch = ctypes.create_string_buffer(64)
    call('fd_device_info', device, ctypes.byref(cu), ctypes.byref(khz), ctypes.byref(mem),
         arch, 64)
    return {'cu_count': cu.value, 'clock_khz': khz.value, 'hbm_bytes': mem.value,
            'arch': arch.value.decode()}


class Plan():

    def __init__(self):
        h = c_void_p()
        call('fd_plan_create', ctypes.byref(h))
        self._h = h
        self._replay = lib().fd_plan_replay

    def record(self):
        import contextlib
# ... 71 lines not shown
```

### flexdiffuse_amd/ops.py

```python
from __future__ import annotations

import ctypes
import os
from ctypes import c_float, c_int32, c_int64, c_void_p
from dataclasses import dataclass
from typing import Optional, Tuple

import torch

from . import hip

ACT_NONE, ACT_SILU, ACT_QUICK_GELU, ACT_GELU, ACT_GEGLU = 0, 1, 2, 3, 4
FAMILY_GEMM, FAMILY_ATTENTION, FAMILY_GROUPNORM, FAMILY_OTHER = 0, 1, 2, 3


class fd_gemm_desc(ctypes.Structure):
    _fields_ = [('A', c_void_p), ('W', c_void_p), ('C', c_void_p), ('bias', c_void_p),
                ('bias2', c_void_p), ('residual', c_void_p),
                ('M', c_int32), ('N', c_int32), ('K', c_int32),
                ('lda', c_int32), ('ldw', c_int32), ('ldc', c_int32), ('ldr', c_int32),
                ('ld_bias2', c_int32), ('rows_per_sample', c_int32), ('act', c_int32),
                ('out_f32', c_int32), ('alpha', c_float),
                ('conv', c_int32), ('in_h', c_int32), ('in_w', c_int32), ('in_c', c_int32),
                ('out_h', c_int32), ('out_w', c_int32), ('kh', c_int32), ('kw', c_int32),
# ... 154 lines not shown
def conv3x3_narrow(x: torch.Tensor, w: NarrowConvW, out: Optional[torch.Tensor] = None, out2: Optional[torch.Tensor] = None,
                   rep2: int = 0, scale: float = 1.0) -> Act:
    B, C, H, W = x.shape
    assert C == w.cin and x.dtype == torch.float32
    x = x.contiguous()
    if out is None:
        out = _empty((B * H * W, w.cout), torch.float16, x)
    assert out.shape == (B * H * W, w.cout) and out.stride(1) == 1 and out.dtype == torch.float16
    if rep2:
        assert out2 is not None and out2.shape == (rep2 * B * H * W, w.cout) and out2.stride(1) == 1 and out2.dtype == torch.float16
    hip.call('fd_conv3x3_narrow_f16', x.data_ptr(), w.w.data_ptr(), _p(w.bias), out.data_ptr(), out.stride(0),
             _p(out2) if rep2 else None, out2.stride(0) if rep2 else 0, rep2, B, C, H, W, w.cout, scale, hip.stream())
    return Act(out, B, H, W)


def prep_conv_shortcut(w: torch.Tensor, b: Optional[torch.Tensor], ws: torch.Tensor, bs: Optional[torch.Tensor],
                       dev) -> ConvW:
    cout, cin, kh, kw = w.shape
    cx = ws.shape[1]
    assert cin % 64 == 0 and cx % 64 == 0 and ws.shape[0] == cout
    k = kh * kw * cin
    wd = torch.zeros((cout, k + cx), dtype=torch.float16, device=dev)
    wd[:, :k] = w.permute(0, 2, 3, 1).reshape(cout, k).to(dev, torch.float16)
    wd[:, k:] = ws.reshape(cout, cx).to(dev, torch.float16)
    bias = (b.float() if b is not None else 0.0) + (bs.float() if bs is not None else 0.0)
    return ConvW(wd, _bias(bias if torch.is_tensor(bias) else None, dev), cout, cin, kh, kw, False, k, cx)


def prep_conv_up_phases(w: torch.Tensor, b: Optional[torch.Tensor], dev) -> ConvW:
    cout, cin, kh, kw = w.shape
    assert kh == 3 and kw == 3 and cin % 64 == 0
    w32 = w.float()
    rows = {0: (w32[:, :, 0:1].sum(2), w32[:, :, 1:3].sum(2)), 1: (w32[:, :, 0:2].sum(2), w32[:, :, 2:3].sum(2))}
    out = torch.zeros((4, cout, 2, 2, cin), dtype=torch.float32)
    for py in (0, 1):
        for a in (0, 1):
            r = rows[py][a]
            cols = {0: (r[:, :, 0:1].sum(2), r[:, :, 1:3].sum(2)), 1: (r[:, :, 0:2].sum(2), r[:, :, 2:3].sum(2))}
            for px in (0, 1):
                for bb in (0, 1):
                    out[py * 2 + px, :, a, bb, :] = cols[px][bb]
    wd = out.reshape(4, cout, 4 * cin).to(dev, torch.float16).contiguous()
    cw = ConvW(wd, _bias(b, dev), cout, cin, 2, 2, False, 4 * cin)
    return cw


def conv2d_up_phases(x: Act, w: ConvW, out: Optional[torch.Tensor] = None) -> Act:
    assert x.C == w.cin and w.w.dim() == 3 and w.w.shape[0] == 4 and x.t.is_contiguous()
    M = x.B * x.H * x.W
    Ho, Wo = 2 * x.H, 2 * x.W
    if out is None:
        out = _empty((x.B * Ho * Wo, w.cout), torch.float16, x.t)
    assert out.shape == (x.B * Ho * Wo, w.cout) and out.stride(1) == 1
    d = fd_gemm_desc()
    d.A, d.W, d.C = x.t.data_ptr(), w.w.data_ptr(), out.data_ptr()
    d.bias = _p(w.bias)
    d.M, d.N, d.K = M, w.cout, w.kpad
    d.ldw, d.ldc = w.w.stride(1), out.stride(0)
    d.rows_per_sample, d.alpha = x.H * x.W, 1.0
    d.conv, d.in_h, d.in_w, d.in_c, d.out_h, d.out_w, d.kh, d.kw = 1, x.H, x.W, w.cin, x.H, x.W, 2, 2
    d.stride, d.pad_t, d.pad_l, d.upsample2x = 1, 1, 1, 2
    d.batch, d.batch_stride_w = 4, w.w.stride(0)
    _sched(d, x.t.device)
    hip.call('fd_gemm_f16', ctypes.byref(d), hip.stream())
    return Act(out, x.B, Ho, Wo)


def up_phases_supported(rows_low: int, cout: int, cin: int) -> bool:
    return (os.environ.get('FD_UP_PHASES', '1') != '0' and rows_low % 256 == 0
            and rows_low >= int(os.environ.get('FD_UP_PHASES_MIN_ROWS', '1024' if cout % 160 == 0 and cout >= 1280 and cin >= 1280 else '4096'))
            and (cout % 160 == 0 or cout % 128 == 0) and cin % 64 == 0)


def f32(t: torch.Tensor, dev) -> torch.Tensor:
    return t.to(dev, torch.float32).contiguous()


def f16(t: torch.Tensor, dev) -> torch.Tensor:
    return t.to(dev, torch.float16).contiguous()


@dataclass
class Act:
    t: torch.Tensor
    B: int
    H: int
    W: int

    @property
    def C(self) -> int:
        return self.t.shape[1]

    @property
    def HW(self) -> int:
        return self.H * self.W


def _empty(shape, dtype, like: torch.Tensor) -> torch.Tensor:
    return torch.empty(shape, dtype=dtype, device=like.device)


_splitk_ws = {}
SPLITK_WS_BYTES = 96 << 20
GN_FINISH_FUSE = os.environ.get('FD_GN_FINISH_FUSE', '1') != '0'
_last_conv_gn_fused = False
gn_fused_launches = 0
FORCE_TILE = 0
FORCE_SPLIT = 0
WS_SLOT = 0


SPLITK_INLAUNCH = os.environ.get('FD_SPLITK_INLAUNCH', '0') == '1'
_sk_sync = {}


def _sched(d: 'fd_gemm_desc', dev: torch.device):
    key = (dev.index if dev.index is not None else 0, WS_SLOT)
    ws = _splitk_ws.get(key)
    if ws is None:
        ws = torch.empty(SPLITK_WS_BYTES, dtype=torch.uint8, device=dev)
        _splitk_ws[key] = ws
    d.workspace, d.workspace_bytes = ws.data_ptr(), SPLITK_WS_BYTES
    d.tile, d.split_k = FORCE_TILE, FORCE_SPLIT


def _inlaunch_request(d: 'fd_gemm_desc', dev: torch.device, tile: int, split: int) -> bool:
    if not SPLITK_INLAUNCH or split <= 1 or tile not in (30, 32):
        return False
    bm = 256 if tile == 30 else 128
    if d.N % 320 or d.M % bm or (d.M // bm) * (d.N // 320) * split > 256 or bm % split:
        return False
    key = (dev.index if dev.index is not None else 0, WS_SLOT)
    t = _sk_sync.get(key)
    if t is None:
        t = torch.zeros(8192, dtype=torch.int32, device=dev)
        _sk_sync[key] = t
    d.sk_sync = t.data_ptr()
    return True


LN_PARTS = os.environ.get('FD_UNET_LN_FINALIZE', '0') != '1'


def _set_ln_stats(d: 'fd_gemm_desc', ln_stats: torch.Tensor, w: LinW, M: int, eps: float = 1e-5):
    assert w.colsum is not None and ln_stats.dtype == torch.float32 and ln_stats.is_contiguous()
    if ln_stats.dim() == 3:
        assert ln_stats.shape[1:] == (M, 2) and ln_stats.shape[0] in (2, 4, 8), tuple(ln_stats.shape)
        d.ln_stats_parts, d.ln_stats_rows, d.ln_fold_eps = ln_stats.shape[0], M, eps
    else:
        assert ln_stats.shape == (M, 2)
    d.ln_stats, d.ln_colsum = ln_stats.data_ptr(), w.colsum.data_ptr()


def gemm(a: torch.Tensor, w: LinW, *, act: int = ACT_NONE, residual: Optional[torch.Tensor] = None,
         bias2: Optional[torch.Tensor] = None, ld_bias2: int = 0, rows_per_sample: int = 0,
         out_f32: bool = False, out: Optional[torch.Tensor] = None, alpha: float = 1.0,
         use_bias: bool = True, ln_stats: Optional[torch.Tensor] = None,
         ln_stats_out: Optional[torch.Tensor] = None, ln_eps: float = 1e-5,
         a2: Optional[torch.Tensor] = None, gn_parts: int = 0):
    M, K = a.shape
    K2 = 0 if a2 is None else a2.shape[1]
    assert a.dtype == torch.float16 and a.stride(1) == 1 and K + K2 == w.K, (a.shape, K2, w.K)
    n_out = w.N // 2 if act == ACT_GEGLU else w.N
    if out is None:
        out = _empty((M, _round_up(n_out, 4)), torch.float32 if out_f32 else torch.float16, a)
    d = fd_gemm_desc()
    d.A, d.W, d.C = a.data_ptr(), w.w.data_ptr(), out.data_ptr()
    d.bias = _p(w.bias) if use_bias else None
    d.bias2 = _p(bias2)
    d.residual = _p(residual)
    d.M, d.N, d.K = M, w.N, K
    d.lda, d.ldw, d.ldc = a.stride(0), w.w.stride(0), out.stride(0)
    d.ldr = residual.stride(0) if residual is not None else 0
    if residual is not None and residual.shape[0] != M:
        assert M % residual.shape[0] == 0, (M, residual.shape)
        d.residual_rows = residual.shape[0]
    d.ld_bias2 = ld_bias2
    d.rows_per_sample = rows_per_sample
    d.act, d.out_f32, d.alpha = act, int(out_f32), alpha
    d.batch = 1
    if a2 is not None:
        assert a2.shape[0] == M and a2.stride(1) == 1 and a2.dtype == torch.float16
        d.A2, d.lda2, d.K2 = a2.data_ptr(), a2.stride(0), K2
    if ln_stats is not None:
        _set_ln_stats(d, ln_stats, w, M)
    if ln_stats_out is not None:
        assert ln_stats_out.shape[-2:] == (M, 2) and ln_stats_out.dtype == torch.float32 and ln_stats_out.is_contiguous()
        d.ln_stats_out, d.ln_eps = ln_stats_out.data_ptr(), ln_eps
    _sched(d, a.device)
    if gn_parts:
        parts = _gn_parts_request(d, M // rows_per_sample, gn_parts, a) if rows_per_sample > 0 and M % rows_per_sample == 0 else None
        hip.call('fd_gemm_f16', ctypes.byref(d), hip.stream())
        return out, parts
    hip.call('fd_gemm_f16', ctypes.byref(d), hip.stream())
    return out


def gemm_vt(a: torch.Tensor, w: LinW, B: int, rows_per_sample: int, ld: int,
            out: Optional[torch.Tensor] = None, ln_stats: Optional[torch.Tensor] = None) -> torch.Tensor:
    M, K = a.shape
    assert M == B * rows_per_sample and K == w.K
    if out is not None:
        assert out.shape == (B, w.N, ld) and out.is_contiguous()
    elif ld == rows_per_sample:
        out = _empty((B, w.N, ld), torch.float16, a)
    else:
        out = torch.zeros((B, w.N, ld), dtype=torch.float16, device=a.device)
    d = fd_gemm_desc()
    d.A, d.W, d.C = a.data_ptr(), w.w.data_ptr(), out.data_ptr()
    d.bias = _p(w.bias)
    d.M, d.N, d.K = M, w.N, K
    d.lda, d.ldw, d.ldc = a.stride(0), w.w.stride(0), 0
    d.rows_per_sample = rows_per_sample
    d.trans_out, d.trans_ld, d.trans_sample_stride = 1, ld, w.N * ld
    d.alpha, d.batch = 1.0, 1
    if ln_stats is not None:
        _set_ln_stats(d, ln_stats, w, M)
    hip.call('fd_gemm_f16', ctypes.byref(d), hip.stream())
    return out


QKV_MERGE = os.environ.get('FD_UNET_QKV', '1') != '0'


def qkv_merge_supported(M: int, C: int, rows_per_sample: int) -> bool:
    return QKV_MERGE and M % 128 == 0 and C % 160 == 0 and rows_per_sample % 32 == 0 and M % rows_per_sample == 0


def gemm_qkv(a: torch.Tensor, w: LinW, B: int, rows_per_sample: int, ln_stats: torch.Tensor) -> Tuple[torch.Tensor, torch.Tensor]:
    M, K = a.shape
    C = w.N // 3
    assert w.N == 3 * C and K == w.K and M == B * rows_per_sample and w.colsum is not None
    qk = _empty((M, 2 * C), torch.float16, a)
    vt = _empty((B, C, rows_per_sample), torch.float16, a)
    d = fd_gemm_desc()
    d.A, d.W, d.C, d.C2 = a.data_ptr(), w.w.data_ptr(), qk.data_ptr(), vt.data_ptr()
    d.bias = _p(w.bias)
    d.M, d.N, d.K = M, w.N, K
    d.lda, d.ldw, d.ldc = a.stride(0), w.w.stride(0), 2 * C
    d.rows_per_sample, d.alpha, d.batch = rows_per_sample, 1.0, 1
    d.trans_n0, d.trans_ld, d.trans_sample_stride = 2 * C, rows_per_sample, C * rows_per_sample
    _set_ln_stats(d, ln_stats, w, M)
    hip.call('fd_gemm_f16', ctypes.byref(d), hip.stream())
    return qk, vt


def bgemm(a: torch.Tensor, w: torch.Tensor, alpha: float = 1.0) -> torch.Tensor:
    Bz, M, K = a.shape
    N = w.shape[1]
    out = _empty((Bz, M, N), torch.float16, a)
    d = fd_gemm_desc()
    d.A, d.W, d.C = a.data_ptr(), w.data_ptr(), out.data_ptr()
    d.M, d.N, d.K = M, N, K
    d.lda, d.ldw, d.ldc = a.stride(1), w.stride(1), N
    d.alpha, d.batch = alpha, Bz
    d.batch_stride_a, d.batch_stride_w, d.batch_stride_c = a.stride(0), w.stride(0), M * N
    hip.call('fd_gemm_f16', ctypes.byref(d), hip.stream())
    return out


@dataclass
class GNSpec:
    gamma: torch.Tensor
    beta: torch.Tensor
    G: int
    eps: float
    silu: bool


@dataclass
class GNParts:
    t: torch.Tensor
    chunks: int
    G: int


GN_PARTS = os.environ.get('FD_GN_PARTS', '1') != '0'


def _gn_parts_request(d: 'fd_gemm_desc', B: int, G: int, like: torch.Tensor) -> Optional[GNParts]:
    if not GN_PARTS or d.act != ACT_NONE or d.out_f32:
        return None
    d.gn_groups = G
    chunks = hip.lib().fd_gemm_gn_parts_chunks(ctypes.byref(d))
    if chunks <= 0:
        return None
    t = _empty((B, chunks, G, 2), torch.float32, like)
    d.gn_part_out, d.gn_part_chunks = t.data_ptr(), chunks
    return GNParts(t, chunks, G)


def conv2d(x: Act, w: ConvW, *, stride: int = 1, pad: Tuple[int, int] = (1, 1), up: bool = False,
           out_hw: Optional[Tuple[int, int]] = None, act: int = ACT_NONE,
           residual: Optional[torch.Tensor] = None, bias2: Optional[torch.Tensor] = None,
           ld_bias2: int = 0, out_f32: bool = False, out: Optional[torch.Tensor] = None,
           a2: Optional[torch.Tensor] = None, gn: Optional[GNSpec] = None, keep: bool = True, gn_parts: int = 0):
    assert x.C == w.cin, (x.C, w.cin)
    Hv, Wv = (x.H * 2, x.W * 2) if up else (x.H, x.W)
    if out_hw is None:
        Ho = (Hv + 2 * pad[0] - w.kh) // stride + 1
        Wo = (Wv + 2 * pad[1] - w.kw) // stride + 1
    else:
        Ho, Wo = out_hw
    M = x.B * Ho * Wo
    if out is None:
        out = _empty((M, _round_up(w.cout, 4)), torch.float32 if out_f32 else torch.float16, x.t)
    assert out.shape == (M, _round_up(w.cout, 4)) and out.stride(1) == 1
    assert x.t.stride(1) == 1 and (x.t.is_contiguous() or (not w.im2col and x.t.stride(0) % 8 == 0 and x.t.data_ptr() % 16 == 0)), \
        'conv input must be an NHWC matrix with unit channel stride (contiguous for the explicit-im2col path)'
    d = fd_gemm_desc()
    d.W, d.C = w.w.data_ptr(), out.data_ptr()
    d.bias, d.bias2, d.residual = _p(w.bias), _p(bias2), _p(residual)
    d.M, d.N, d.K = M, w.cout, w.kpad
    d.ldw, d.ldc = w.w.stride(0), out.stride(0)
    d.ldr = residual.stride(0) if residual is not None else 0
    d.ld_bias2, d.rows_per_sample = ld_bias2, Ho * Wo
    d.act, d.out_f32, d.alpha, d.batch = act, int(out_f32), 1.0, 1
    if w.im2col:
        if up:
            raise ValueError(f'conv2d: the fused nearest-2x upsample needs Cin % 64 == 0 (got {w.cin}): the explicit-im2col '
                             'path of narrow inputs has no upsample form')
        cols = _empty((M, w.kpad), torch.float16, x.t)
        hip.call('fd_im2col_f16', x.t.data_ptr(), cols.data_ptr(), x.B, x.H, x.W, w.cin, Ho, Wo,
                 w.kh, w.kw, stride, pad[0], pad[1], w.kpad, hip.stream())
        d.A, d.lda = cols.data_ptr(), w.kpad
    else:
        d.A, d.lda = x.t.data_ptr(), x.t.stride(0)
        d.conv, d.in_h, d.in_w, d.in_c = 1, x.H, x.W, w.cin
        d.out_h, d.out_w, d.kh, d.kw = Ho, Wo, w.kh, w.kw
        d.stride, d.pad_t, d.pad_l, d.upsample2x = stride, pad[0], pad[1], int(up)
    k2 = w.k2
    if k2:
        assert a2 is not None and not w.im2col and a2.shape == (M, k2) and a2.stride(1) == 1 and a2.dtype == torch.float16
        d.A2, d.lda2, d.K2 = a2.data_ptr(), a2.stride(0), k2
    else:
        assert a2 is None
    _sched(d, x.t.device)
    if gn is not None:
        lib = hip.lib()
        tile, split = c_int32(0), c_int32(0)
        hip.check(lib.fd_gemm_plan(ctypes.byref(d), ctypes.byref(tile), ctypes.byref(split)), 'fd_gemm_plan')
        inl = _inlaunch_request(d, x.t.device, tile.value, split.value)
        fuse = (not inl and GN_FINISH_FUSE and split.value > 1 and act == ACT_NONE and not out_f32 and w.cout % 8 == 0 and out.stride(0) % 8 == 0
                and (residual is None or (residual.stride(0) % 8 == 0 and residual.data_ptr() % 16 == 0))
                and (bias2 is None or (ld_bias2 % 4 == 0 and bias2.data_ptr() % 16 == 0))
                and lib.fd_gemm_can_fuse_groupnorm(M, w.cout, Ho * Wo, gn.G, split.value))
        global _last_conv_gn_fused, gn_fused_launches
        _last_conv_gn_fused = bool(fuse)
        gn_fused_launches += int(bool(fuse))
        if not fuse:
            parts = _gn_parts_request(d, x.B, gn.G, x.t)
            hip.call('fd_gemm_f16', ctypes.byref(d), hip.stream())
            res = Act(out, x.B, Ho, Wo)
            return res, groupnorm(res, gn.gamma, gn.beta, gn.G, gn.eps, gn.silu, parts=parts)
        y = _empty((M, w.cout), torch.float16, x.t)
        d.gn_out, d.gn_gamma, d.gn_beta = y.data_ptr(), gn.gamma.data_ptr(), gn.beta.data_ptr()
        d.gn_groups, d.gn_silu, d.gn_eps, d.gn_skip_c = gn.G, int(gn.silu), gn.eps, int(not keep)
        hip.call('fd_gemm_f16', ctypes.byref(d), hip.stream())
        return (Act(out, x.B, Ho, Wo) if keep else None), Act(y, x.B, Ho, Wo)
    if SPLITK_INLAUNCH and act == ACT_NONE and not out_f32:
        tile, split = c_int32(0), c_int32(0)
        hip.check(hip.lib().fd_gemm_plan(ctypes.byref(d), ctypes.byref(tile), ctypes.byref(split)), 'fd_gemm_plan')
        _inlaunch_request(d, x.t.device, tile.value, split.value)
    if gn_parts:
        parts = _gn_parts_request(d, x.B, gn_parts, x.t)
        hip.call('fd_gemm_f16', ctypes.byref(d), hip.stream())
        return Act(out, x.B, Ho, Wo), parts
    hip.call('fd_gemm_f16', ctypes.byref(d), hip.stream())
    return Act(out, x.B, Ho, Wo)


QK_LOG2E = 1.4426950408889634


def attention_accepts_prescaled(head_dim: int) -> bool:
    return os.environ.get('FD_ATTN_QT1', '2') == '2' and (head_dim <= 80 or head_dim > 128)


def attention(q: torch.Tensor, k: torch.Tensor, vt: torch.Tensor, B: int, heads: int, n_q: int,
              n_k: int, head_dim: int, causal: bool = False, q_prescaled: bool = False,
              out: Optional[torch.Tensor] = None) -> torch.Tensor:
    if out is None:
        out = _empty((B * n_q, heads * head_dim), torch.float16, q)
    assert out.shape == (B * n_q, heads * head_dim) and out.dtype == torch.float16
    d = fd_attention_desc()
    d.Q, d.K, d.Vt, d.O = q.data_ptr(), k.data_ptr(), vt.data_ptr(), out.data_ptr()
    d.ldq, d.ldk, d.ldvt, d.ldo = q.stride(0), k.stride(0), vt.stride(1), out.stride(0)
    d.q_sample_stride, d.k_sample_stride = n_q * q.stride(0), n_k * k.stride(0)
    d.vt_sample_stride, d.o_sample_stride = vt.stride(0), n_q * out.stride(0)
    d.batch, d.heads, d.n_q, d.n_k, d.head_dim = B, heads, n_q, n_k, head_dim
    d.causal, d.scale, d.q_prescaled = int(causal), 0.0, int(q_prescaled)
    hip.call('fd_attention_f16', ctypes.byref(d), hip.stream())
    return out


class fd_xattn_desc(ctypes.Structure):
# ... 658 lines not shown
```

### flexdiffuse_amd/unet.py

```python
from __future__ import annotations

import os
from types import SimpleNamespace
from typing import Dict, List, Optional

import torch

from . import hip, ops
from .ops import Act
from .weights import SD15_UNET, UNetConfig, unet_param_shapes, unet_up_plan


class _Res:
    def __init__(self, sd, name, dev, temb_off):
        self.n1g, self.n1b = ops.f32(sd[name + '.norm1.weight'], dev), ops.f32(sd[name + '.norm1.bias'], dev)
        self.n2g, self.n2b = ops.f32(sd[name + '.norm2.weight'], dev), ops.f32(sd[name + '.norm2.bias'], dev)
        self.conv1 = ops.prep_conv(sd[name + '.conv1.weight'], sd[name + '.conv1.bias'], dev)
        self.conv2 = ops.prep_conv(sd[name + '.conv2.weight'], sd[name + '.conv2.bias'], dev)
        self.short = None
        self.sc_fused = False
        if name + '.conv_shortcut.weight' in sd:
            w = sd[name + '.conv_shortcut.weight']
            w2 = sd[name + '.conv2.weight']
            if os.environ.get('FD_UNET_SC_FUSE', '1') != '0' and w.shape[1] % 64 == 0 and w2.shape[1] % 64 == 0:
# ... 159 lines not shown
        return plan

    def set_attention_slice(self, slice_size):
        self.attention_slice = slice_size

    def to(self, device):
        return self

    def __call__(self, sample, timestep, encoder_hidden_states=None, return_dict=True):
        return self.forward(sample, timestep, encoder_hidden_states)

    def set_context(self, ctx: torch.Tensor):
        key = (ctx.data_ptr(), ctx._version, tuple(ctx.shape))
        if key == self._ctx_key:
            return
        hip.require_device(ctx)
        if self._ctx_sched is not None:
            self._ctx_sched = None
            for a in self._attn_layers:
                a.ctx_kv, a.ctx_img, a.ctx_fold = None, None, None
        Be, L, D = ctx.shape
        c16 = ops.cast_f16(ctx.reshape(Be * L, D)) if ctx.dtype != torch.float16 \
            else ctx.reshape(Be * L, D).contiguous()
        ldv = (L + 7) // 8 * 8
        realloc = False
        for a in self._attn_layers:
            old = a.ctx_kv
            if old is not None and old[0].shape == (Be * L, a.C) and old[1].shape == (Be, a.C, ldv):
                ops.gemm(c16, a.k2, out=old[0])
                ops.gemm_vt(c16, a.v2, Be, L, ldv, out=old[1])
            else:
                a.ctx_kv = (ops.gemm(c16, a.k2), ops.gemm_vt(c16, a.v2, Be, L, ldv), L)
                a.ctx_img, a.ctx_fold = None, None
                realloc = True
            if a.ln_fold and a.q_pre and ops.xattn_supported(a.heads, a.C // a.heads, L, ops.xattn_row_tile(a.C // a.heads)):
                a.ctx_img = ops.xattn_pack_kv(a.ctx_kv[0], a.ctx_kv[1], Be, L, a.heads, a.C // a.heads, out=a.ctx_img)
            else:
                a.ctx_img = None
            if a.q2t is not None and ops.xattn_fold_layer(a.C, a.heads, L):
                f = a.ctx_fold
                kf, vf = ops.xattn_fold(a.ctx_kv[0], ops.gemm(c16, a.v2), a.q2t, a.o2.w, Be, L, a.heads, out=None if f is None else (f.kf, f.vf))
                a.ctx_fold = ops.XFold(kf, vf, ops.xattn_fold_rows(kf, a.ctx_kv[0], a.q2.bias, L, a.heads, out=None if f is None else f.rows), L)
                realloc = realloc or f is None
            else:
                a.ctx_fold = None
        if realloc:
            self.ctx_generation += 1
        self._ctx_key = key
        self._ctx_ref = ctx

    def _ctx_layout(self, Be: int, L: int):
        ldv = (L + 7) // 8 * 8
        up = lambda n: (n + 7) // 8 * 8
        off, slots = 0, []
        for a in self._attn_layers:
            d = a.C // a.heads
            ok, off = off, off + up(Be * L * a.C)
            ov, off = off, off + up(Be * a.C * ldv)
            oi, nb = None, 0
            if a.ln_fold and a.q_pre and ops.xattn_supported(a.heads, d, L, ops.xattn_row_tile(d)):
                nb = hip.lib().fd_xattn_image_bytes(a.heads, d)
                oi = (off, off + up(Be * nb // 2))
                off = oi[1] + up(Be * nb // 2)
            of = None
            if a.q2t is not None and ops.xattn_fold_layer(a.C, a.heads, L):
                n = Be * a.heads * ops.XF_GROUP * a.C
                of = (off, off + up(n))
                off = of[1] + up(n)
            slots.append((ok, ov, oi, nb, of))
        return off, slots

    @staticmethod
    def _ctx_views(arena: torch.Tensor, slot, Be: int, L: int, C: int):
        ok, ov, oi, nb = slot[:4]
        ldv = (L + 7) // 8 * 8
        kv = (arena[ok:ok + Be * L * C].view(Be * L, C), arena[ov:ov + Be * C * ldv].view(Be, C, ldv), L)
        img = None if oi is None else tuple(arena[o:o + Be * nb // 2].view(torch.uint8).view(Be, nb) for o in oi)
        return kv, img

    @staticmethod
    def _ctx_fold_views(arena: torch.Tensor, slot, Be: int, a: _Attn):
        if slot[4] is None:
            return None
        N, n = a.heads * ops.XF_GROUP, Be * a.heads * ops.XF_GROUP * a.C
        return arena[slot[4][0]:slot[4][0] + n].view(Be, N, a.C), arena[slot[4][1]:slot[4][1] + n].view(Be, a.C, N)

    def set_context_keyframes(self, ctxs) -> torch.Tensor:
        from .ctx_schedule import check_keyframes
        Be, L, D = check_keyframes(ctxs)
        key = tuple((c.data_ptr(), c._version, tuple(c.shape)) for c in ctxs)
        sch = self._ctx_sched
        if sch is not None and sch['key'] == key:
            return sch['handle']
        hip.require_device(*ctxs)
        total, slots = self._ctx_layout(Be, L)
        if sch is None or sch['shape'] != (len(ctxs), Be, L, D):
            arenas = [torch.zeros((total,), dtype=torch.float16, device=self.device) for _ in range(len(ctxs) + 1)]
            sch = {'shape': (len(ctxs), Be, L, D), 'arenas': arenas,
                   'handle': torch.zeros((Be, L, D), dtype=torch.float16, device=self.device)}
            for a, slot in zip(self._attn_layers, slots):
                a.ctx_kv, a.ctx_img = self._ctx_views(arenas[-1], slot, Be, L, a.C)
                fv = self._ctx_fold_views(arenas[-1], slot, Be, a)
                a.ctx_fold = None if fv is None else ops.XFold(fv[0], fv[1], torch.zeros((Be, 2, fv[0].shape[1]), dtype=torch.float32, device=self.device), L)
            self.ctx_generation += 1
        ldv = (L + 7) // 8 * 8
        for ctx, arena in zip(ctxs, sch['arenas']):
            c16 = ops.cast_f16(ctx.reshape(Be * L, D)) if ctx.dtype != torch.float16 else ctx.reshape(Be * L, D).contiguous()
            for a, slot in zip(self._attn_layers, slots):
                kv, img = self._ctx_views(arena, slot, Be, L, a.C)
                ops.gemm(c16, a.k2, out=kv[0])
                ops.gemm_vt(c16, a.v2, Be, L, ldv, out=kv[1])
                if img is not None:
                    ops.xattn_pack_kv(kv[0], kv[1], Be, L, a.heads, a.C // a.heads, out=img)
                fv = self._ctx_fold_views(arena, slot, Be, a)
                if fv is not None:
                    ops.xattn_fold(kv[0], ops.gemm(c16, a.v2), a.q2t, a.o2.w, Be, L, a.heads, out=fv)
        sch['key'], sch['refs'], sch['live'] = key, list(ctxs), None
        self._ctx_sched = sch
        h = sch['handle']
        self._ctx_key, self._ctx_ref = (h.data_ptr(), h._version, tuple(h.shape)), h
        self.blend_context(0, 0.0)
        return h

    def context_buffers(self, i: int = -1):
        sch = self._ctx_sched
        if sch is None:
            raise RuntimeError('context_buffers needs set_context_keyframes first (the UNet is not in schedule mode)')
        _, Be, L, _ = sch['shape']
        slots = self._ctx_layout(Be, L)[1]
        return [self._ctx_views(sch['arenas'][i], slot, Be, L, a.C) for a, slot in zip(self._attn_layers, slots)]

    def blend_context(self, k: int, w: float):
        sch = self._ctx_sched
        if sch is None:
            raise RuntimeError('blend_context needs set_context_keyframes first (the UNet is not in schedule mode)')
        arenas = sch['arenas']
        if not 0 <= k < len(arenas) - 2:
            raise ValueError(f'segment {k} of {len(arenas) - 1} keyframes')
        if sch['live'] == (k, float(w)):
            return
        ops.lerp_f16(arenas[k], arenas[k + 1], float(w), out=arenas[-1])
        for a in self._attn_layers:
            if a.ctx_fold is not None:
                ops.xattn_fold_rows(a.ctx_fold.kf, a.ctx_kv[0], a.q2.bias, a.ctx_fold.L, a.heads, out=a.ctx_fold.rows)
        sch['live'] = (k, float(w))

    @staticmethod
    def _qkv_level(M: int) -> bool:
        lo, hi = os.environ.get('FD_UNET_QKV_MIN_ROWS'), os.environ.get('FD_UNET_QKV_MAX_ROWS')
        if lo is not None or hi is not None:
            return int(lo or 0) <= M <= int(hi or (1 << 30))
        return not (8192 <= M <= 16384)

    def _gn1(self, r: Optional[_Res]) -> Optional[ops.GNSpec]:
        return None if r is None else ops.GNSpec(r.n1g, r.n1b, self.G, 1e-5, True)

    def _attn_gn(self, a: Optional[_Attn], x: Act):
        if a is None:
            return None
        if ops.gn_fold_supported(x.B, x.HW, a.C, a.C, self.G):
            return self.G
        return ops.GNSpec(a.ng, a.nb, self.G, 1e-6, False)

    def _res(self, r: _Res, x: Act, temb: torch.Tensor, out: Optional[torch.Tensor] = None, xn: Optional[Act] = None,
             next_gn=None):
        if isinstance(xn, Act):
            h = xn
        else:
            h = ops.groupnorm(x, r.n1g, r.n1b, self.G, 1e-5, True, parts=xn)
        _, h = ops.conv2d(h, r.conv1, bias2=temb[:, r.temb_off:r.temb_off + r.cout], ld_bias2=self.temb_total,
                          gn=ops.GNSpec(r.n2g, r.n2b, self.G, 1e-5, True), keep=False)
        kw = dict(a2=x.t) if r.sc_fused else dict(residual=x.t if r.short is None else ops.gemm(x.t, r.short))
        if next_gn is None:
            return ops.conv2d(h, r.conv2, out=out, **kw), None
        if isinstance(next_gn, int):
            return ops.conv2d(h, r.conv2, out=out, gn_parts=next_gn, **kw)
        return ops.conv2d(h, r.conv2, out=out, gn=next_gn, keep=True, **kw)

    def _attn(self, a: _Attn, x: Act, rep: int = 1, out: Optional[torch.Tensor] = None, xn=None, next_parts: int = 0):
        B, HW, C = x.B, x.HW, a.C
        d = C // a.heads
        gn_fold = ops.gn_fold_supported(B, HW, C, C, self.G)
        h = None if gn_fold else (xn if isinstance(xn, Act) else ops.groupnorm(x, a.ng, a.nb, self.G, 1e-6, False))
        emit = (a.ln_fold and a.ln_emit) and ops.can_emit_row_stats(B * HW, C, C)

        def mkst(rows, batch=1):
            k = emit and ops.can_emit_row_stats(rows, C, C)
            if not k:
                return None
            return torch.empty((rows * batch, 2) if k == 1 else (k, rows * batch, 2), dtype=torch.float32, device=x.t.device)

        def fin(st, hh, parts_ok=False):
            if st is None:
                return ops.ln_row_stats(hh)
            if st.dim() == 2 or (parts_ok and ops.LN_PARTS and st.shape[0] in (2, 4, 8)):
                return st
            return ops.ln_finalize_stats(st, C)
        if gn_fold:
            wb, bb = ops.gn_fold_linear(x, a.gnf, parts=xn if isinstance(xn, ops.GNParts) else None)
            st = mkst(HW, B)
            h = ops.gemm_per_sample(x.t, wb, bb, B, HW, ln_stats_out=st)
        else:
            st = mkst(B * HW)
            h = ops.gemm(h.t, a.proj_in, ln_stats_out=st)
        if a.ln_fold:
            st = fin(st, h, parts_ok=True)
            if a.qkv1 is not None and ops.qkv_merge_supported(B * HW, C, HW) and self._qkv_level(B * HW):
                qk, vt = ops.gemm_qkv(h, a.qkv1, B, HW, st)
            else:
                qk = ops.gemm(h, a.qk1, ln_stats=st)
                vt = ops.gemm_vt(h, a.v1, B, HW, (HW + 7) // 8 * 8, ln_stats=st)
        else:
            n = ops.layernorm(h, *a.ln[0])
            qk = ops.gemm(n, a.qk1)
            vt = ops.gemm_vt(n, a.v1, B, HW, (HW + 7) // 8 * 8)
        q, k = qk[:, :C], qk[:, C:]
        o = ops.attention(q, k, vt, B, a.heads, HW, HW, d, q_prescaled=a.q_pre)
        st = mkst(B * HW)
        h = ops.gemm(o, a.o1, residual=h, ln_stats_out=st)
        kc, vtc, L = a.ctx_kv
        xt = x.t
        fold = a.ctx_fold if ops.XATTN_FOLD and rep == 1 and a.ctx_fold is not None and a.ctx_fold.kf.shape[0] == B else None
        if fold is not None:
            nparts = st.shape[0] if st is not None and st.dim() == 3 and ops.LN_PARTS and st.shape[0] in (2, 4, 8) else 0
            if not ops.xattn_fold_plan(B, HW, C, a.heads, L, parts=nparts):
                fold = None
        if fold is not None:
            p = ops.xattn_fold_probs(h, fold, fin(st, h, parts_ok=True), B, HW, L)
            ns = ops.xattn_fold_out_slabs(B, HW, C, p.shape[1]) if emit else 0
            st = torch.empty((ns, B * HW, 2), dtype=torch.float32, device=p.device) if ns > 1 else None
            h = ops.xattn_fold_out(p, fold, a.o2.bias, h, B, HW, ln_stats_out=st)
        elif a.ctx_img is not None and HW % ops.xattn_row_tile(d) == 0:
            o = ops.xattn_q(h, a.q2, fin(st, h, parts_ok=True), a.ctx_img, HW, L, a.heads, d, n_rep=rep)
        else:
            if a.ln_fold:
                q2 = ops.gemm(h, a.q2, ln_stats=fin(st, h, parts_ok=True))
            else:
                q2 = ops.gemm(ops.layernorm(h, *a.ln[1]), a.q2)
            if rep == 1:
                o = ops.attention(q2, kc, vtc, B, a.heads, HW, L, d, q_prescaled=a.q_pre)
            else:
                o = torch.empty((rep * B * HW, C), dtype=torch.float16, device=q2.device)
                for r in range(rep):
                    ops.attention(q2, kc[r * B * L:(r + 1) * B * L], vtc[r * B:(r + 1) * B], B, a.heads,
                                  HW, L, d, q_prescaled=a.q_pre, out=o[r * B * HW:(r + 1) * B * HW])
        if fold is not None:
            pass
        elif rep > 1:
            if not ops.residual_wrap_supported(B * HW, rep):
                h, xt = ops.repeat_rows(h, rep), ops.repeat_rows(xt, rep)
            B = rep * B
        if fold is None:
            st = mkst(B * HW)
            h = ops.gemm(o, a.o2, residual=h, ln_stats_out=st)
        if a.ln_fold:
            f = ops.gemm(h, a.ff1, act=ops.ACT_GEGLU, ln_stats=fin(st, h, parts_ok=C >= 1280))
        else:
            f = ops.gemm(ops.layernorm(h, *a.ln[2]), a.ff1, act=ops.ACT_GEGLU)
        if a.ffp is not None:
            if next_parts:
                o, parts = ops.gemm(f, a.ffp, a2=h, residual=xt, out=out, rows_per_sample=HW, gn_parts=next_parts)
                return Act(o, B, x.H, x.W), parts
            return Act(ops.gemm(f, a.ffp, a2=h, residual=xt, out=out), B, x.H, x.W)
        h = ops.gemm(f, a.ff2, residual=h)
        res = Act(ops.gemm(h, a.proj_out, residual=xt, out=out), B, x.H, x.W)
        return (res, None) if next_parts else res

    def time_bias(self, timestep, B: int) -> torch.Tensor:
        dev = self.device
        if isinstance(timestep, torch.Tensor):
            t = timestep.to(dev, torch.float32).reshape(-1)
            if t.numel() not in (1, B):
                raise ValueError(f'timestep tensor has {t.numel()} elements for a batch of {B}')
            t = t.contiguous()
        else:
            t = torch.full((1,), float(timestep), dtype=torch.float32, device=dev)
        dim = self.cfg.block_out_channels[0]
        e = torch.empty((B, dim), dtype=torch.float16, device=dev)
        hip.call('fd_timestep_embedding_f16', t.data_ptr(), 0 if t.numel() == 1 else 1, e.data_ptr(), B, dim,
                 hip.stream())
        e = ops.gemm(e, self.t1, act=ops.ACT_SILU)
        e = ops.gemm(e, self.t2, act=ops.ACT_SILU)
        return ops.gemm(e, self.temb_all, out_f32=True)

    def time_bias_table(self, timesteps) -> torch.Tensor:
        t = torch.tensor([float(v) for v in timesteps], dtype=torch.float32, device=self.device)
        return self.time_bias(t, t.numel())

    def forward_nhwc(self, sample: torch.Tensor, timestep, ctx: torch.Tensor,
                     rep: int = 1, temb: Optional[torch.Tensor] = None) -> torch.Tensor:
        hip.require_device(sample, ctx)
        self.set_context(ctx)
        share = rep > 1 and (temb is not None or not isinstance(timestep, torch.Tensor) or timestep.numel() == 1)
        direct = ops.CONV_IN_DIRECT and self.conv_in_nw is not None and (share or rep == 1) and sample.shape[3] <= 1024
        x = None if direct else ops.nchw_to_nhwc(sample, rep=1 if share else rep, c_pad=self.conv_in.cin)
        xB, xH, xW = (sample.shape[0], sample.shape[2], sample.shape[3]) if direct else (x.B, x.H, x.W)
        Be = xB * (rep if share else 1)
        if ctx.shape[0] != Be:
            raise ValueError(f'encoder_hidden_states batch {ctx.shape[0]} != latent batch {Be}')
        if temb is None:
            temb = self.time_bias(timestep, Be)
        elif temb.shape != (Be, self.temb_total) or temb.dtype != torch.float32 or not temb.is_contiguous():
            raise ValueError(f'temb must be a contiguous fp32 [{Be}][{self.temb_total}] tensor, got {tuple(temb.shape)} {temb.dtype}')
        fan = rep if share else 1
        plan = self._cat_plan
        skips: List[tuple] = []

        def slot(rows: int, cs: int):
            ch = plan[len(skips)] if len(skips) < len(plan) else None
            if ch is None:
                return None, None, None
            buf = torch.empty((rows, ch + cs), dtype=torch.float16, device=self.device)
            return buf, buf[:, ch:], ch

        def push(act: Act, buf, ch):
            skips.append((act, buf, ch))
            return act

        def left(rows: int, c: int):
            if skips and skips[-1][1] is not None and skips[-1][2] == c and skips[-1][1].shape[0] == rows:
                return skips[-1][1][:, :c]
            return None

        HW = xH * xW
        buf, view, ch = slot(Be * HW, self.conv_in.cout)
        if direct and fan > 1:
            rep_out = view if view is not None else torch.empty((Be * HW, self.conv_in.cout), dtype=torch.float16, device=self.device)
            h = ops.conv3x3_narrow(sample.to(torch.float32), self.conv_in_nw, out2=rep_out, rep2=fan)
            push(Act(rep_out, Be, xH, xW), buf if view is not None else None, ch if view is not None else None)
        elif direct:
            h = push(ops.conv3x3_narrow(sample.to(torch.float32), self.conv_in_nw, out=view), buf, ch)
        elif fan > 1:
            h = ops.conv2d(x, self.conv_in)
            if view is None:
                push(Act(ops.repeat_rows(h.t, fan), Be, h.H, h.W), None, None)
            else:
                ops.repeat_rows(h.t, fan, out=view)
                push(Act(view, Be, h.H, h.W), buf, ch)
        else:
            h = push(ops.conv2d(x, self.conv_in, out=view), buf, ch)
        pend: Optional[Act] = None
        seq = [r for blk in self.down for r in blk['res']] + [self.mid_res0]
        nres = 0
        for blk in self.down:
            for r, a in zip(blk['res'], blk['attn']):
                rows = Be * h.H * h.W
                buf, view, ch = slot(rows, r.cout)
                nres += 1
                if a is not None:
                    h, hn = self._res(r, h, temb[:h.B], xn=pend, next_gn=self._attn_gn(a, h))
                    if r is not blk['res'][-1]:
                        h, pend = self._attn(a, h, fan, out=view, xn=hn, next_parts=self.G)
                    else:
                        h, pend = self._attn(a, h, fan, out=view, xn=hn), None
                elif fan > 1:
                    h, pend = self._res(r, h, temb[:h.B], xn=pend)
                    if view is None:
                        h = Act(ops.repeat_rows(h.t, fan), Be, h.H, h.W)
                    else:
                        ops.repeat_rows(h.t, fan, out=view)
                        h = Act(view, Be, h.H, h.W)
                else:
                    nxt = seq[nres] if blk['down'] is None or r is not blk['res'][-1] else None
                    h, pend = self._res(r, h, temb[:h.B], out=view, xn=pend, next_gn=self._gn1(nxt))
                fan = 1
                push(h, buf, ch)
            if blk['down'] is not None:
                buf, view, ch = slot(Be * (h.H // 2) * (h.W // 2), blk['down'].cout)
                if blk['down'].im2col:
                    h, pend = ops.conv2d(h, blk['down'], stride=2, out=view), None
                else:
                    h, pend = ops.conv2d(h, blk['down'], stride=2, out=view, gn=self._gn1(seq[nres]), keep=True)
                push(h, buf, ch)
        h, hn = self._res(self.mid_res0, h, temb, xn=pend, next_gn=self._attn_gn(self.mid_attn, h))
        h = self._attn(self.mid_attn, h, xn=hn)
        h, _ = self._res(self.mid_res1, h, temb, out=left(h.B * h.HW, self.mid_res1.cout))
        out_parts = None
        for blk in self.up:
            n = len(blk['res'])
            for j, (r, a) in enumerate(zip(blk['res'], blk['attn'])):
                s, sbuf, sch = skips.pop()
                if sbuf is not None and h.t.data_ptr() == sbuf.data_ptr() and h.C == sch:
                    h = Act(sbuf, h.B, h.H, h.W)
                else:
                    h = Act(ops.concat_channels(ops.contiguous_rows(h.t), ops.contiguous_rows(s.t)), h.B, h.H, h.W)
                last = j == n - 1
                dst = None if (last and blk['up'] is not None) else left(h.B * h.HW, r.cout)
                if a is not None:
                    h, hn = self._res(r, h, temb, next_gn=self._attn_gn(a, h))
                    if last and blk['up'] is None:
                        h, out_parts = self._attn(a, h, out=dst, xn=hn, next_parts=self.G)
                    else:
                        h = self._attn(a, h, out=dst, xn=hn)
                else:
                    h, _ = self._res(r, h, temb, out=dst)
            if blk['up'] is not None:
                dst = left(h.B * h.HW * 4, blk['up'].cout)
                if blk.get('up_ph') is not None and h.t.is_contiguous() and ops.up_phases_supported(h.B * h.HW, blk['up'].cout, blk['up'].cin):
                    h = ops.conv2d_up_phases(h, blk['up_ph'], out=dst)
                else:
                    h = ops.conv2d(h, blk['up'], up=True, out=dst)
        h = ops.groupnorm(h, self.out_g, self.out_b, self.G, 1e-5, True, parts=out_parts)
        return ops.conv2d(h, self.conv_out, out_f32=True).t

    def forward(self, sample, timestep, encoder_hidden_states) -> UNetOutput:
        B, C, H, W = sample.shape
        eps = self.forward_nhwc(sample, timestep, encoder_hidden_states)
        return UNetOutput(sample=ops.nhwc_to_nchw(eps, B, self.cfg.out_channels, H, W))
```

### include/flexdiffuse_hip.h

```cpp
#ifndef FLEXDIFFUSE_HIP_H
#define FLEXDIFFUSE_HIP_H

#include <stdint.h>

#ifdef __cplusplus
extern "C" {
#endif

#define FD_OK 0
#define FD_EINVAL (-1)
#define FD_ESHAPE (-2)
#define FD_EHIP (-3)

#define FD_ABI_VERSION 12

int fd_abi_version(void);
const char* fd_last_error(void);
int fd_device_info(int device, int* cu_count, int* clock_khz, int64_t* hbm_bytes,
                   char* arch, int arch_len);

#define FD_FAMILY_GEMM 0
#define FD_FAMILY_ATTENTION 1
#define FD_FAMILY_GROUPNORM 2
#define FD_FAMILY_OTHER 3
int fd_prof_enable(int on);
int fd_prof_set_stride(int stride);
int fd_prof_collect(int family, double* total_ms, double* total_work, int64_t* launches);
int fd_prof_collect2(int family, double* total_ms, double* total_work, double* total_executed, int64_t* launches);
int fd_prof_drain(int32_t* family, uint32_t* tag, float* ms, double* work, double* executed, int64_t cap, int64_t* n);
int fd_prof_calibrate(int pairs, double* ms_per_empty_pair, void* stream);

typedef struct fd_plan fd_plan;
int fd_plan_create(fd_plan** out);
int fd_plan_destroy(fd_plan* plan);
int fd_plan_record_begin(fd_plan* plan);
int fd_plan_record_end(fd_plan* plan);
int fd_plan_size(const fd_plan* plan, int* launches);
int fd_plan_replay(const fd_plan* plan, void* stream);

#define FD_ORDER_TEXT 0
#define FD_ORDER_ALIGN 1
#define FD_ORDER_DIRECT 2

int64_t fd_guidance_workspace_floats(int B, int N, int L);

int fd_guidance_map(const float* alt, const float* txt, float* ws, int32_t* idx, float* s,
                    int B, int alt_batched, int N, int L, int D, int order, int reuse,
                    void* stream);

typedef struct fd_tween_params {
    double threshold_floor;
    double threshold_mult;
    double clustered;
    double max_guidance;
    double header_max;
    int32_t order;
    int32_t reuse;
} fd_tween_params;

int fd_guidance_tween(const float* base, const float* alt, const float* lin_w, float* ws,
                      float* out, float* weights, int32_t* idx, float* s, int32_t* status,
                      int B, int alt_batched, int N, int L, int D,
                      const fd_tween_params* p, void* stream);

int fd_guidance_concept_override(const float* guide, const int32_t* cm_idx,
                                 const int32_t* ct_idx, const float* ct_s, float* out,
                                 int N, int L, int D, void* stream);

int fd_guidance_header_pull(float* out, const float* hdr, int B, int L, int D, void* stream);

#define FD_ACT_NONE 0
#define FD_ACT_SILU 1
#define FD_ACT_QUICK_GELU 2
#define FD_ACT_GELU 3
#define FD_ACT_GEGLU 4

typedef struct fd_gemm_desc {
    const void* A;
    const void* W;
    void* C;
    const float* bias;
    const float* bias2;
    const void* residual;
    int32_t M, N, K;
    int32_t lda, ldw, ldc, ldr, ld_bias2;
    int32_t rows_per_sample;
    int32_t act;
    int32_t out_f32;
    float alpha;
    int32_t conv, in_h, in_w, in_c, out_h, out_w, kh, kw, stride, pad_t, pad_l, upsample2x;
    int32_t trans_out, trans_ld;
    int64_t trans_sample_stride;
    int32_t batch;
    int64_t batch_stride_a, batch_stride_w, batch_stride_c, batch_stride_res;
    int32_t tile, split_k;
    void* workspace;
    int64_t workspace_bytes;
    const float* ln_stats;
    const float* ln_colsum;
    float* ln_stats_out;
    float ln_eps;
    const void* A2;
    int32_t lda2, K2;
    int64_t batch_stride_bias;
    void* gn_out;
    const float* gn_gamma;
    const float* gn_beta;
    int32_t gn_groups, gn_silu;
    float gn_eps;
    int32_t gn_skip_c;
    float* gn_part_out;
    int32_t gn_part_chunks;
    int32_t trans_n0;
    void* C2;
    void* sk_sync;
    int32_t ln_stats_parts, ln_stats_rows;
    float ln_fold_eps;
    int32_t residual_rows;
    int32_t softmax_group, softmax_valid;
} fd_gemm_desc;

int fd_gemm_f16(const fd_gemm_desc* desc, void* stream);
int fd_gemm_can_emit_row_stats(int M, int N, int K, int ldc, int ldr);
int fd_gemm_plan(const fd_gemm_desc* d, int* tile, int* split_k);
int fd_gemm_can_fuse_groupnorm(int M, int N, int rows_per_sample, int groups, int split_k);
int fd_gemm_gn_parts_chunks(const fd_gemm_desc* d);
int fd_xattn_fold_rows_f32(const void* kf, const void* K, const float* bias_q, float* rows, int samples, int n_keys, int heads, int head_dim,
                           int C, int ldk, void* stream);

typedef struct fd_attention_desc {
    const void* Q;
    const void* K;
    const void* Vt;
    void* O;
    int64_t q_sample_stride, k_sample_stride, vt_sample_stride, o_sample_stride;
    int32_t ldq, ldk, ldvt, ldo;
    int32_t batch, heads, n_q, n_k, head_dim;
    int32_t causal;
    float scale;
    int32_t q_prescaled;
} fd_attention_desc;

int fd_attention_f16(const fd_attention_desc* desc, void* stream);

int64_t fd_xattn_image_bytes(int heads, int head_dim);
int fd_xattn_pack_kv_f16(const void* K, const void* Vt, void* k_image, void* v_image, int samples, int n_keys,
                         int heads, int head_dim, int ldk, int ldvt, int64_t k_sample_stride,
                         int64_t vt_sample_stride, void* stream);
typedef struct fd_xattn_desc {
    const void* x;
    const void* wq;
    const float* bias;
    const float* ln_colsum;
    const float* ln_stats;
    const void* k_image;
    const void* v_image;
    void* out;
    int32_t M, ldx, ldw, ldo;
    int32_t rows_per_sample;
    int32_t n_rep;
    int32_t n_keys, heads, head_dim;
    int32_t ln_stats_parts;
    float ln_fold_eps;
} fd_xattn_desc;
int fd_xattn_q_f16(const fd_xattn_desc* desc, void* stream);

int64_t fd_groupnorm_workspace_floats(int B, int G);
int fd_groupnorm_nhwc_f16(const void* x, void* y, const float* gamma, const float* beta,
                          float* ws, int B, int HW, int C, int G, float eps, int silu,
                          void* stream);
int fd_groupnorm_nhwc_ld_f16(const void* x, int ldx, void* y, const float* gamma, const float* beta,
                             float* ws, int B, int HW, int C, int G, float eps, int silu,
                             void* stream);
int fd_groupnorm_apply_parts_f16(const void* x, int ldx, void* y, const float* gamma, const float* beta, const float* parts,
                                 int chunks, int B, int HW, int C, int G, float eps, int silu, void* stream);
int fd_groupnorm_fold_linear_f16(const void* x, int ldx, float* ws, int B, int HW, int C, int G, float eps,
                                 const void* wg, const float* biasf, int N,
                                 void* w_out, float* bias_out, void* stream);
int fd_groupnorm_fold_linear_parts_f16(const float* parts, int chunks, int B, int HW, int C, int G, float eps,
                                       const void* wg, const float* biasf, int N, void* w_out, float* bias_out, void* stream);
int fd_layernorm_f16(const void* x, void* y, const float* gamma, const float* beta, int rows,
                     int C, int ldx, int ldy, float eps, int out_f32, void* stream);
int fd_ln_row_stats_f16(const void* x, float* stats, int rows, int C, int ldx, float eps, void* stream);
int fd_ln_finalize_stats_f32(const float* partials, float* stats, int M, int N, int n_tiles, float eps, void* stream);
int fd_softmax_rows_f16(void* x, int rows, int N, int ld, float scale, void* stream);

int fd_nchw_f32_to_nhwc_f16(const float* x, void* y, int B, int C, int HW, int rep, int c_pad,
                            float scale, void* stream);
int fd_nhwc_f32_to_nchw_f32(const float* x, float* y, int B, int C, int HW, int ld, float a,
                            float b, int clamp01, void* stream);
int fd_conv3x3_narrow_f16(const float* x, const void* w, const float* bias, void* y, int ldy, void* y2, int ldy2, int rep2,
                          int B, int Cin, int H, int W, int Cout, float scale, void* stream);
int fd_im2col_f16(const void* x, void* y, int B, int Hi, int Wi, int Cin, int Ho, int Wo, int KH,
                  int KW, int stride, int pad_t, int pad_l, int k_pad, void* stream);
int fd_concat_channels_f16(const void* a, const void* b, void* out, int64_t M, int Ca, int Cb,
                           void* stream);
int fd_cfg_ddim_step_f32(float* x, const float* eps_nhwc, float* eps_out, int B, int C, int HW,
                         int ld, int cfg, float guidance, float c1, float c2, float c3, float c4,
                         int v_prediction, int do_step, void* stream);
int fd_axpby_f32(const float* x, const float* y, float* out, int64_t n, float a, float b,
                 int exp_half_x, void* stream);
int fd_embed_tokens_f16(const int64_t* ids, const void* tok_emb, const void* pos_emb, void* out,
                        int B, int L, int D, int vocab, void* stream);
int fd_vit_assemble_f16(const void* patches, const void* cls, const void* pos, void* out, int B,
                        int T, int D, void* stream);
int fd_timestep_embedding_f16(const float* t, int t_stride, void* out, int B, int dim, void* stream);
int fd_copy2d_f16(const void* src, int lds, void* dst, int ldd, int64_t rows, int cols, void* stream);
int fd_repeat_rows_f16(const void* src, int lds, void* dst, int ldd, int64_t rows, int cols, int rep, void* stream);
int fd_region_blend_f32(float* dst, const float* src, int C, int H, int W, int oy, int ox, int sh,
                        int sw, float blend, void* stream);
int fd_composite_step_f32(float* x, const float* eps_nhwc, const float* weights, float* eps_out, int B, int C,
                          int HW, int ld, int n_entities, int cfg, float guidance, float c1, float c2, float c3,
                          float c4, int v_prediction, int do_step, void* stream);
int fd_cfg_ddim_masked_step_f32(float* x, const float* eps_nhwc, const float* z0, const float* noise, const float* mask,
                                int B, int C, int HW, int ld, int cfg, float guidance, float c1, float c2, float c3,
                                float c4, int v_prediction, float k1, float k2, void* stream);
int fd_cfg_multistep_step_f32(float* x, const float* eps_nhwc, float* m0_out, const float* m1, const float* z0,
                              const float* noise, const float* mask, int B, int C, int HW, int ld, int cfg, float guidance,
                              float p, float q, float a, float w0, float w1, float k1, float k2, void* stream);
int fd_cfg_linear_multistep_step_f32(float* x, const float* eps_nhwc, int form, int n_prev, const float* h1, const float* h2,
                                     const float* h3, float* h_out, float* x_keep_out, const float* x_src,
                                     float* x_scaled_out, const float* z0, const float* noise, const float* mask, int B, int C,
                                     int HW, int ld, int cfg, float guidance, float w0, float w1, float w2, float w3, float a0,
                                     float a1, float a2, float scale, float k1, float k2, void* stream);
int fd_philox_normal_f32(float* out, int64_t n, int per, uint64_t seed, int64_t sample_offset, int draw, int noise_stream,
                         void* stream);
int fd_cfg_ddim_noise_step_f32(float* x, const float* eps_nhwc, const float* z0, const float* noise, const float* mask,
                               int B, int C, int HW, int ld, int cfg, float guidance, float c1, float c2, float c3,
                               float c4, int v_prediction, float k1, float k2, float sigma, uint64_t seed,
                               int64_t sample_offset, int per, int draw, void* stream);
int fd_cfg_multistep_noise_step_f32(float* x, const float* eps_nhwc, float* m0_out, const float* m1, const float* z0,
                                    const float* noise, const float* mask, int B, int C, int HW, int ld, int cfg,
                                    float guidance, float p, float q, float a, float w0, float w1, float k1, float k2,
                                    float sn, uint64_t seed, int64_t sample_offset, int per, int draw, void* stream);
int fd_cfg_rescale_ddim_step_f32(float* x, const float* eps_nhwc, float* eps_out, float* scale_out, const float* z0,
                                 const float* noise, const float* mask, int B, int C, int HW, int ld, float guidance,
                                 float rescale, float c1, float c2, float c3, float c4, int v_prediction, int do_step,
                                 float k1, float k2, float sigma, uint64_t seed, int64_t sample_offset, int draw,
                                 void* stream);
int fd_cfg_rescale_multistep_step_f32(float* x, const float* eps_nhwc, float* m0_out, const float* m1, float* scale_out,
                                      const float* z0, const float* noise, const float* mask, int B, int C, int HW, int ld,
                                      float guidance, float rescale, float p, float q, float a, float w0, float w1,
                                      float k1, float k2, float sn, uint64_t seed, int64_t sample_offset, int draw,
                                      void* stream);
int fd_composite_ddim_step_f32(float* x, const float* eps_nhwc, const float* weights, int n_entities, float* eps_out,
                               const float* z0, const float* noise, const float* mask, int B, int C, int HW, int ld, int cfg,
                               float guidance, float c1, float c2, float c3, float c4, int v_prediction, float k1, float k2,
                               float sigma, uint64_t seed, int64_t sample_offset, int per, int draw, void* stream);
int fd_composite_multistep_step_f32(float* x, const float* eps_nhwc, const float* weights, int n_entities, float* m0_out,
                                    const float* m1, const float* z0, const float* noise, const float* mask, int B, int C,
                                    int HW, int ld, int cfg, float guidance, float p, float q, float a, float w0, float w1,
                                    float k1, float k2, float sn, uint64_t seed, int64_t sample_offset, int per, int draw,
                                    void* stream);
int fd_composite_linear_multistep_step_f32(float* x, const float* eps_nhwc, const float* weights, int n_entities, int form,
                                           int n_prev, const float* h1, const float* h2, const float* h3, float* h_out,
                                           float* x_keep_out, const float* x_src, float* x_scaled_out, const float* z0,
                                           const float* noise, const float* mask, int B, int C, int HW, int ld, int cfg,
                                           float guidance, float w0, float w1, float w2, float w3, float a0, float a1, float a2,
                                           float scale, float k1, float k2, void* stream);
int fd_lerp_f16(const void* a, const void* b, void* out, int64_t n, float w, void* stream);
int fd_window_gather_f32(const float* canvas, float* windows, int B, int C, int H, int W, int h, int w, int stride_y,
                         int stride_x, int ny, int nx, void* stream);
int fd_window_step_f32(float* x, float* windows_out, const float* eps_nhwc, float* eps_out, int B, int C, int ld, int H,
                       int W, int h, int w, int stride_y, int stride_x, int ny, int nx, int blend, int cfg, float guidance,
                       float c1, float c2, float c3, float c4, int v_prediction, int do_step, void* stream);
int fd_window_ddim_step_f32(float* x, float* windows_out, const float* eps_nhwc, float* eps_out, const float* z0,
                            const float* noise, const float* mask, int B, int C, int ld, int H, int W, int h, int w,
                            int stride_y, int stride_x, int ny, int nx, int blend, int cfg, float guidance, float c1, float c2,
                            float c3, float c4, int v_prediction, float k1, float k2, float sigma, uint64_t seed,
                            int64_t sample_offset, int draw, void* stream);
int fd_window_multistep_step_f32(float* x, float* windows_out, const float* eps_nhwc, float* m0_out, const float* m1,
                                 const float* z0, const float* noise, const float* mask, int B, int C, int ld, int H, int W,
                                 int h, int w, int stride_y, int stride_x, int ny, int nx, int blend, int cfg, float guidance,
                                 float p, float q, float a, float w0, float w1, float k1, float k2, float sn, uint64_t seed,
                                 int64_t sample_offset, int draw, void* stream);
int fd_cast_f32_to_f16(const float* x, void* y, int64_t n, void* stream);
int fd_cast_f16_to_f32(const void* x, float* y, int64_t n, void* stream);

#ifdef __cplusplus
// ... 4 lines not shown
```

Baseline: 10.94 images/sec.

## Add row-resident K=320 GEMM kernel for LN-folded QKV projection

Adds a new GEMM kernel specialised for K=320. Each wave keeps its 32 rows of A in registers and streams 32-column weight chunks through a multi-stage LDS ring filled by buffer-to-LDS DMA, with LayerNorm-fold and GEGLU or transposed-V epilogues. It is enabled by default for the merged QKV projection at M=65536/32768. The GEGLU path is wired up, but its level table is empty, so it stays off. It also fixes the per-device attribute flag so it is set only after hipFuncSetAttribute succeeds; this adds a load/fetch_or split that is not atomic as one step.

```diff
diff --git a/flexdiffuse_amd/csrc/common.h b/flexdiffuse_amd/csrc/common.h
--- a/flexdiffuse_amd/csrc/common.h
+++ b/flexdiffuse_amd/csrc/common.h
@@ -70,11 +70,14 @@
 
 #ifdef __cplusplus
 #include <atomic>
-static inline bool fd_first_on_device(std::atomic<unsigned long long>* mask) {
+static inline bool fd_first_on_device(const std::atomic<unsigned long long>* mask) {
     int dev = 0;
     if (hipGetDevice(&dev) != hipSuccess) return true;
-    const unsigned long long bit = 1ull << (dev & 63);
-    return (mask->fetch_or(bit) & bit) == 0;
+    return (mask->load() & (1ull << (dev & 63))) == 0;
+}
+static inline void fd_done_on_device(std::atomic<unsigned long long>* mask) {
+    int dev = 0;
+    if (hipGetDevice(&dev) == hipSuccess) mask->fetch_or(1ull << (dev & 63));
 }
 #endif
 
diff --git a/flexdiffuse_amd/csrc/gemm.hip b/flexdiffuse_amd/csrc/gemm.hip
--- a/flexdiffuse_amd/csrc/gemm.hip
+++ b/flexdiffuse_amd/csrc/gemm.hip
@@ -870,8 +870,10 @@
     size_t lds = 0;
     const int GB = gn_slab_pick<256, 16>(g.rows_per_batch, g.N, g.gn_groups, &lds);
     static std::atomic<unsigned long long> configured{0};
-    if (lds > 64 * 1024 && fd_first_on_device(&configured))
+    if (lds > 64 * 1024 && fd_first_on_device(&configured)) {
         FD_HIP(hipFuncSetAttribute(reinterpret_cast<const void*>(k_splitk_finish_gn<S>), hipFuncAttributeMaxDynamicSharedMemorySize, 160 * 1024));
+        fd_done_on_device(&configured);
+    }
     hipLaunchKernelGGL(k_splitk_finish_gn<S>, dim3(g.M / g.rows_per_batch, g.gn_groups / GB), dim3(256), lds, st, g);
     FD_CHECK_LAUNCH("k_splitk_finish_gn");
     return FD_OK;
@@ -921,6 +923,7 @@
             if constexpr (BN != 320 && EPI != 13 && EPI != 14)
                 FD_HIP(hipFuncSetAttribute(reinterpret_cast<const void*>(k_gemm_f16_dmap<BM, BN, CONV, WM, TRANS, WN, EPI>),
                                            hipFuncAttributeMaxDynamicSharedMemorySize, (int)lds));
+            fd_done_on_device(&configured);
         }
         const int occ = (BM >= 256 || lds > 80 * 1024) ? 1 : (BM * BN >= 128 * 128) ? 2 : (BM == 128 ? 3 : 4);
         const int slots = 256 * occ;
@@ -958,9 +961,11 @@
         return FD_ESHAPE;
     } else {
         static std::atomic<unsigned long long> configured{0};
-        if (lds > 64 * 1024 && fd_first_on_device(&configured))
+        if (lds > 64 * 1024 && fd_first_on_device(&configured)) {
             FD_HIP(hipFuncSetAttribute(reinterpret_cast<const void*>(k_gemm_f16<BM, BN, TRANS, CONV>),
                                        hipFuncAttributeMaxDynamicSharedMemorySize, (int)lds));
+            fd_done_on_device(&configured);
+        }
         hipLaunchKernelGGL((k_gemm_f16<BM, BN, TRANS, CONV>), grid, dim3(256), lds, st, g);
         FD_CHECK_LAUNCH("k_gemm_f16");
         return FD_OK;
diff --git a/flexdiffuse_amd/csrc/gemm_pp.hip b/flexdiffuse_amd/csrc/gemm_pp.hip
--- a/flexdiffuse_amd/csrc/gemm_pp.hip
+++ b/flexdiffuse_amd/csrc/gemm_pp.hip
@@ -425,9 +425,11 @@
                                             : 2ull * ((unsigned long long)(g.M - 1) * g.lda + g.K);
     const unsigned long long w_bytes = 2ull * ((unsigned long long)(g.N - 1) * g.ldw + g.K + g.K2);
     static std::atomic<unsigned long long> configured{0};
-    if (fd_first_on_device(&configured))
+    if (fd_first_on_device(&configured)) {
         FD_HIP(hipFuncSetAttribute(reinterpret_cast<const void*>(k_gemm_f16_pp<WM_, WN_, MI, NI, CONV, EPI, HAS_K2>),
                                    hipFuncAttributeMaxDynamicSharedMemorySize, (int)lds));
+        fd_done_on_device(&configured);
+    }
     static const int sk_xcd = getenv("FD_PP_SK_XCD") ? atoi(getenv("FD_PP_SK_XCD")) : 1;
     const int nb = g.tiles_m * g.tiles_n;
     g.sk_flat = sk_xcd && (g.split_k == 2 || g.split_k == 4 || g.split_k == 8) && batch == 1 && nb % (8 / g.split_k) == 0 &&
diff --git a/flexdiffuse_amd/csrc/gemm_rowres.hip b/flexdiffuse_amd/csrc/gemm_rowres.hip
--- /dev/null
+++ b/flexdiffuse_amd/csrc/gemm_rowres.hip
@@ -0,0 +1,304 @@
+#include "gemm_epilogue.h"
+
+typedef __attribute__((address_space(3))) void* lds_ptr;
+
+#define RR_K 320
+#define RR_BN 32
+#define RR_W_BYTES (RR_BN * RR_K * 2)
+#define RR_STAGE (RR_W_BYTES + 1024)
+#define RR_LDS_BYTES(WAVES, ST) ((ST) * RR_STAGE + (WAVES) * 32 * 8)
+
+struct RowresArgs {
+    const half_t* A;
+    const half_t* W;
+    half_t* C;
+    half_t* C2;
+    const float* bias;
+    const float* colsum;
+    const float* stats;
+    int M, N, lda, ldw, ldc;
+    int tr_n0, rows_per_batch, ldt;
+    long long strideT;
+    unsigned w_bytes;
+};
+
+template <int FORM, int WAVES, int ST>
+__global__ __launch_bounds__(WAVES * 64) __attribute__((amdgpu_waves_per_eu(2, 2))) void k_gemm_rowres(RowresArgs g) {
+#if defined(__HIP_DEVICE_COMPILE__)
+    static_assert((WAVES == 4 || WAVES == 8) && ST >= 3, "4 or 8 waves, a ring of at least 3 stages");
+    constexpr int S = FORM == 0 ? 1 : 2;
+    constexpr int RR_ROWS = WAVES * 32;
+    constexpr int RR_DMAS = WAVES == 4 ? 6 : 3;
+    extern __shared__ __attribute__((aligned(16))) char smem[];
+    const int tid = threadIdx.x, lane = tid & 63;
+    const int wave = __builtin_amdgcn_readfirstlane(tid >> 6);
+    const int r = lane & 31, h = lane >> 5;
+    const int wg_m0 = blockIdx.x * RR_ROWS;
+    const int m0 = wg_m0 + wave * 32;
+    const int nblk = g.N / RR_BN;
+
+    const __amdgpu_buffer_rsrc_t rsW = __builtin_amdgcn_make_buffer_rsrc((void*)g.W, 0, g.w_bytes, 0x00020000);
+    const __amdgpu_buffer_rsrc_t rsB = __builtin_amdgcn_make_buffer_rsrc((void*)(g.bias ? (const void*)g.bias : (const void*)g.W), 0,
+                                                                         g.bias ? (unsigned)g.N * 4u : 0u, 0x00020000);
+    const __amdgpu_buffer_rsrc_t rsCS = __builtin_amdgcn_make_buffer_rsrc((void*)g.colsum, 0, (unsigned)g.N * 4u, 0x00020000);
+
+    float* const stats_s = reinterpret_cast<float*>(smem + ST * RR_STAGE);
+    if (FORM == 1 && tid < RR_ROWS)
+        *reinterpret_cast<floatx2*>(stats_s + 2 * tid) = *reinterpret_cast<const floatx2*>(g.stats + 2 * (size_t)(wg_m0 + tid));
+    const floatx2 st = *reinterpret_cast<const floatx2*>(g.stats + 2 * (size_t)(m0 + r));
+
+    half8 fa[20];
+    {
+        const half_t* ap = g.A + (size_t)(m0 + r) * g.lda + h * 8;
+#pragma unroll
+        for (int ks = 0; ks < 20; ++ks) fa[ks] = *reinterpret_cast<const half8*>(ap + ks * 16);
+    }
+    __builtin_amdgcn_sched_barrier(0);
+
+    const int rsub = lane >> 3;
+    const int grp = wave & 3, upper = wave >> 2;
+    const int key_w = ((rsub >> 1) & 1) | (grp << 1);
+    const unsigned w_lane = (unsigned)(rsub * g.ldw) * 2u + (unsigned)((((lane & 7) ^ key_w)) << 4);
+    constexpr unsigned OOB = 0x80000000u;
+#define RR_ISSUE(CB, SLOT)                                                                                                    \
+    {                                                                                                                         \
+        const int cb_ = (CB);                                                                                                 \
+        const bool ok_ = cb_ < nblk;    \
+        char* dst_ = smem + (SLOT) * RR_STAGE + grp * 1024;                                                                   \
+        const int soff_ = (cb_ * RR_BN + grp * 8) * g.ldw * 2;                                                                \
+        const unsigned wv_ = ok_ ? w_lane : OOB;                                                                              \
+        char* aux_ = smem + (SLOT) * RR_STAGE + RR_W_BYTES + grp * 256;                                                       \
+        const unsigned bv_ = (ok_ && lane < RR_BN) ? (unsigned)lane * 4u : OOB;              \
+        if (WAVES == 4 || !upper) {                                                                                           \
+            _Pragma("unroll") for (int kt = 0; kt < (WAVES == 4 ? 5 : 3); ++kt)                                               \
+                __builtin_amdgcn_raw_ptr_buffer_load_lds(rsW, (lds_ptr)(dst_ + kt * 4096), 16, wv_, soff_ + kt * 128, 0, 0);  \
+        } else {                                                                                                              \
+            _Pragma("unroll") for (int kt = 3; kt < 5; ++kt)                                                                  \
+                __builtin_amdgcn_raw_ptr_buffer_load_lds(rsW, (lds_ptr)(dst_ + kt * 4096), 16, wv_, soff_ + kt * 128, 0, 0);  \
+        }                                                                                                                     \
+        if (WAVES == 4 || upper) {                                                                                            \
+            if (wave & 1) __builtin_amdgcn_raw_ptr_buffer_load_lds(rsCS, (lds_ptr)aux_, 4, bv_, cb_ * RR_BN * 4, 0, 0);       \
+            else __builtin_amdgcn_raw_ptr_buffer_load_lds(rsB, (lds_ptr)aux_, 4, bv_, cb_ * RR_BN * 4, 0, 0);                 \
+        }                                                                                                                     \
+    }
+#define RR_WAIT(N) asm volatile("s_waitcnt vmcnt(%0)" ::"n"(N) : "memory");
+#define RR_BAR()                          \
+    __builtin_amdgcn_sched_barrier(0);    \
+    __builtin_amdgcn_s_barrier();         \
+    __builtin_amdgcn_sched_barrier(0);
+
+#pragma unroll
+    for (int i = 0; i < ST - 1; ++i) RR_ISSUE(i, i)
+    __builtin_amdgcn_sched_barrier(0);
+    RR_WAIT((ST - 2) * RR_DMAS)
+
+    const int key_r = ((r >> 1) & 1) | ((r >> 3) << 1);
+    int rd[4];
+#pragma unroll
+    for (int s = 0; s < 4; ++s) rd[s] = r * 128 + (((2 * s + h) ^ key_r) << 4);
+
+    half_t* const Crow = g.C + (size_t)(m0 + r) * g.ldc + h * 8;
+    const int smp = FORM == 1 ? m0 / g.rows_per_batch : 0;
+    half_t* const Ct = FORM == 1 ? g.C2 + (size_t)smp * g.strideT + (size_t)r * g.ldt + (m0 - smp * g.rows_per_batch) + h * 8 : nullptr;
+    const floatx2 s0 = {st[0], st[0]}, s1 = {st[1], st[1]};
+    typedef const __attribute__((address_space(3))) floatx4* lds_cf4;
+
+    int slot = 0;
+#pragma clang loop unroll(disable)
+    for (int c = 0; c < nblk; ++c) {
+        RR_BAR()
+        {
+            const int sp = slot >= 1 ? slot - 1 : ST - 1;
+            RR_ISSUE(c + ST - 1, sp)
+        }
+        const int cb = c;
+        __builtin_amdgcn_sched_barrier(0);
+        const char* const stg = smem + slot * RR_STAGE;
+        const float* const bias_s = reinterpret_cast<const float*>(stg + RR_W_BYTES);
+        const float* const cs_s = bias_s + 64;
+        floatx16 acc;
+#pragma unroll
+        for (int i = 0; i < 16; ++i) acc[i] = 0.f;
+        const bool tr_blk = FORM == 1 && __builtin_amdgcn_readfirstlane(cb * RR_BN >= g.tr_n0 ? 1 : 0) != 0;
+        if (!tr_blk) {
+#pragma unroll
+            for (int kt = 0; kt < 5; ++kt)
+#pragma unroll
+                for (int s = 0; s < 4; ++s) {
+                    const half8 fb = *reinterpret_cast<const half8*>(stg + kt * 4096 + rd[s]);
+                    acc = __builtin_amdgcn_mfma_f32_32x32x16_f16(fb, fa[kt * 4 + s], acc, 0, 0, 0);
+                }
+            floatx4 bb[4], cc[4];
+#pragma unroll
+            for (int k = 0; k < 4; ++k) {
+                bb[k] = *(lds_cf4)(bias_s + 8 * k + 4 * h);
+                cc[k] = *(lds_cf4)(cs_s + 8 * k + 4 * h);
+            }
+            if constexpr (FORM == 0) {
+                half4 og[2];
+#pragma unroll
+                for (int k = 0; k < 2; ++k)
+#pragma unroll
+                    for (int q = 0; q < 4; q += 2) {
+                        const floatx2 av = {acc[4 * k + q], acc[4 * k + q + 1]};
+                        const floatx2 ag = {acc[4 * (k + 2) + q], acc[4 * (k + 2) + q + 1]};
+                        const floatx2 tv = __builtin_elementwise_fma(s1, floatx2{cc[k][q], cc[k][q + 1]}, floatx2{bb[k][q], bb[k][q + 1]});
+                        const floatx2 tg = __builtin_elementwise_fma(s1, floatx2{cc[k + 2][q], cc[k + 2][q + 1]}, floatx2{bb[k + 2][q], bb[k + 2][q + 1]});
+                        const floatx2 v = __builtin_elementwise_fma(av, s0, tv);
+                        const floatx2 o = v * gelu_fast2(__builtin_elementwise_fma(ag, s0, tg));
+                        og[k][q] = (half_t)o[0];
+                        og[k][q + 1] = (half_t)o[1];
+                    }
+                const u32x2 x = __builtin_bit_cast(u32x2, og[0]), y = __builtin_bit_cast(u32x2, og[1]);
+                const auto p0 = __builtin_amdgcn_permlane32_swap(x[0], y[0], false, false);
+                const auto p1 = __builtin_amdgcn_permlane32_swap(x[1], y[1], false, false);
+                *reinterpret_cast<u32x4*>(Crow + cb * 16) = u32x4{p0[0], p1[0], p0[1], p1[1]};
+            } else {
+                half4 oh[4];
+#pragma unroll
+                for (int k = 0; k < 4; ++k)
+#pragma unroll
+                    for (int q = 0; q < 4; ++q) oh[k][q] = (half_t)fmaf(acc[4 * k + q], st[0], fmaf(st[1], cc[k][q], bb[k][q]));
+#pragma unroll
+                for (int k = 0; k < 4; k += 2) {
+                    const u32x2 x = __builtin_bit_cast(u32x2, oh[k]), y = __builtin_bit_cast(u32x2, oh[k + 1]);
+                    const auto p0 = __builtin_amdgcn_permlane32_swap(x[0], y[0], false, false);
+                    const auto p1 = __builtin_amdgcn_permlane32_swap(x[1], y[1], false, false);
+                    *reinterpret_cast<u32x4*>(Crow + cb * RR_BN + k * 8) = u32x4{p0[0], p1[0], p0[1], p1[1]};
+                }
+            }
+        } else {
+            if constexpr (FORM == 1) {
+#pragma unroll
+                for (int kt = 0; kt < 5; ++kt)
+#pragma unroll
+                    for (int s = 0; s < 4; ++s) {
+                        const half8 fb = *reinterpret_cast<const half8*>(stg + kt * 4096 + rd[s]);
+                        acc = __builtin_amdgcn_mfma_f32_32x32x16_f16(fa[kt * 4 + s], fb, acc, 0, 0, 0);
+                    }
+                const float bn = bias_s[r], cn = cs_s[r];
+                half4 oh[4];
+#pragma unroll
+                for (int k = 0; k < 4; ++k) {
+                    const floatx4 sa = *(lds_cf4)(stats_s + 2 * (wave * 32 + 8 * k + 4 * h));
+                    const floatx4 sb = *(lds_cf4)(stats_s + 2 * (wave * 32 + 8 * k + 4 * h) + 4);
+                    oh[k][0] = (half_t)fmaf(acc[4 * k + 0], sa[0], fmaf(sa[1], cn, bn));
+                    oh[k][1] = (half_t)fmaf(acc[4 * k + 1], sa[2], fmaf(sa[3], cn, bn));
+                    oh[k][2] = (half_t)fmaf(acc[4 * k + 2], sb[0], fmaf(sb[1], cn, bn));
+                    oh[k][3] = (half_t)fmaf(acc[4 * k + 3], sb[2], fmaf(sb[3], cn, bn));
+                }
+                half_t* const Cn = Ct + (size_t)(cb * RR_BN - g.tr_n0) * g.ldt;
+#pragma unroll
+                for (int k = 0; k < 4; k += 2) {
+                    const u32x2 x = __builtin_bit_cast(u32x2, oh[k]), y = __builtin_bit_cast(u32x2, oh[k + 1]);
+                    const auto p0 = __builtin_amdgcn_permlane32_swap(x[0], y[0], false, false);
+                    const auto p1 = __builtin_amdgcn_permlane32_swap(x[1], y[1], false, false);
+                    *reinterpret_cast<u32x4*>(Cn + k * 8) = u32x4{p0[0], p1[0], p0[1], p1[1]};
+                }
+            }
+        }
+        __builtin_amdgcn_sched_barrier(0);
+        if (c < ST - 2) { RR_WAIT((ST - 2) * RR_DMAS + S) } else { RR_WAIT((ST - 2) * RR_DMAS + (ST - 1) * S) }
+        slot = slot == ST - 1 ? 0 : slot + 1;
+    }
+#undef RR_ISSUE
+#undef RR_WAIT
+#undef RR_BAR
+#endif
+}
+
+static int rowres_check(const fd_gemm_desc* d, RowresArgs& g, int* form, int* waves) {
+    FD_CHECK_ARG(d && d->A && d->W && d->C, FD_EINVAL, "fd_gemm_rowres_f16: null pointer");
+    FD_CHECK_ARG(d->M > 0 && d->N > 0 && d->K > 0, FD_EINVAL, "fd_gemm_rowres_f16: M/N/K must be > 0");
+    FD_CHECK_ARG(d->K == RR_K, FD_ESHAPE, "fd_gemm_rowres_f16: K=%d (the row-resident kernel is built for K == 320)", d->K);
+    FD_CHECK_ARG(d->tile >= 0 && d->tile <= 2, FD_ESHAPE, "fd_gemm_rowres_f16: tile=%d (0 = auto, 1 = 128-row, 2 = 256-row workgroups)", d->tile);
+    *waves = d->tile == 2 || (d->tile == 0 && d->M % 256 == 0 && d->M / 256 >= 256) ? 8 : 4;
+    FD_CHECK_ARG(d->M % (*waves * 32) == 0, FD_ESHAPE, "fd_gemm_rowres_f16: M=%d is not a multiple of the workgroup's %d rows", d->M, *waves * 32);
+    FD_CHECK_ARG(d->N % RR_BN == 0, FD_ESHAPE, "fd_gemm_rowres_f16: N=%d is not a multiple of the %d-column chunk", d->N, RR_BN);
+    FD_CHECK_ARG(d->split_k <= 1, FD_ESHAPE, "fd_gemm_rowres_f16: split-K (split_k=%d) is not provided", d->split_k);
+    FD_CHECK_ARG(!d->residual && !d->residual_rows, FD_ESHAPE, "fd_gemm_rowres_f16: a residual is not provided");
+    FD_CHECK_ARG(!d->ln_stats_out, FD_ESHAPE, "fd_gemm_rowres_f16: ln_stats_out is not provided");
+    FD_CHECK_ARG(!d->conv, FD_ESHAPE, "fd_gemm_rowres_f16: convolutions are not provided");
+    FD_CHECK_ARG(d->batch <= 1 && !d->ln_stats_parts, FD_ESHAPE, "fd_gemm_rowres_f16: batch / ln_stats_parts are not provided");
+    FD_CHECK_ARG(!d->bias2 && !d->out_f32 && !d->trans_out && !d->A2 && !d->K2 && !d->gn_out && !d->gn_part_out && !d->sk_sync &&
+                     !d->softmax_group && !d->upsample2x && (d->alpha == 0.f || d->alpha == 1.f),
+                 FD_ESHAPE, "fd_gemm_rowres_f16: only the LayerNorm-fold GEGLU and q|k|v forms are provided (no bias2 / fp32 or transposed output / "
+                            "appended operand / GroupNorm outputs / softmax / alpha)");
+    FD_CHECK_ARG(d->ln_stats && d->ln_colsum, FD_ESHAPE, "fd_gemm_rowres_f16: needs the LayerNorm fold (ln_stats, ln_colsum)");
+    FD_CHECK_ARG(d->lda >= RR_K && d->lda % 8 == 0 && d->ldw >= RR_K && d->ldw % 8 == 0 && d->ldc % 8 == 0, FD_ESHAPE,
+                 "fd_gemm_rowres_f16: lda=%d, ldw=%d must be >= 320 and, like ldc=%d, multiples of 8", d->lda, d->ldw, d->ldc);
+    FD_CHECK_ARG(((uintptr_t)d->A | (uintptr_t)d->W | (uintptr_t)d->C | (uintptr_t)d->bias | (uintptr_t)d->ln_colsum) % 16 == 0 &&
+                     (uintptr_t)d->ln_stats % 8 == 0,
+                 FD_ESHAPE, "fd_gemm_rowres_f16: A, W, C, bias and ln_colsum must be 16-byte aligned, ln_stats 8-byte aligned");
+    const unsigned long long w_bytes = 2ull * ((unsigned long long)(d->N - 1) * d->ldw + RR_K);
+    const unsigned long long a_elems = (unsigned long long)(d->M - 1) * d->lda + RR_K;
+    FD_CHECK_ARG(w_bytes < 0x7ffffff0ull && a_elems < 0x7fffffffull, FD_ESHAPE, "fd_gemm_rowres_f16: operands >= 2 GiB");
+    memset(&g, 0, sizeof(g));
+    if (d->act == FD_ACT_GEGLU && !d->trans_n0) {
+        FD_CHECK_ARG(d->ldc >= d->N / 2 && (unsigned long long)(d->M - 1) * d->ldc + d->N / 2 < 0x7fffffffull, FD_ESHAPE,
+                     "fd_gemm_rowres_f16: GEGLU output row stride ldc=%d < N / 2", d->ldc);
+        *form = 0;
+    } else if (d->act == FD_ACT_NONE && d->trans_n0 > 0) {
+        const int rps = d->rows_per_sample > 0 ? d->rows_per_sample : d->M;
+        FD_CHECK_ARG(d->C2 && (uintptr_t)d->C2 % 16 == 0 && d->trans_n0 % RR_BN == 0 && d->trans_n0 < d->N && rps % 128 == 0 && d->M % rps == 0 &&
+                         d->trans_ld % 8 == 0 && d->trans_ld >= rps && d->trans_sample_stride % 8 == 0 && d->ldc >= d->trans_n0,
+                     FD_ESHAPE, "fd_gemm_rowres_f16: trans_n0 needs C2 (16-byte aligned), trans_n0 %% 32 == 0 and < N, rows_per_sample %% 128 == 0 and | M, "
+                                "trans_ld %% 8 == 0 and >= rows_per_sample, trans_sample_stride %% 8 == 0, ldc >= trans_n0");
+        g.C2 = (half_t*)d->C2;
+        g.tr_n0 = d->trans_n0;
+        g.rows_per_batch = rps;
+        g.ldt = d->trans_ld;
+        g.strideT = d->trans_sample_stride;
+        *form = 1;
+    } else {
+        fd_set_error("fd_gemm_rowres_f16: act=%d trans_n0=%d is neither the GEGLU form (act GEGLU, no trans_n0) nor the q|k|v form (act NONE, trans_n0)",
+                     d->act, d->trans_n0);
+        return FD_ESHAPE;
+    }
+    g.A = (const half_t*)d->A;
+    g.W = (const half_t*)d->W;
+    g.C = (half_t*)d->C;
+    g.bias = d->bias;
+    g.colsum = d->ln_colsum;
+    g.stats = d->ln_stats;
+    g.M = d->M; g.N = d->N; g.lda = d->lda; g.ldw = d->ldw; g.ldc = d->ldc;
+    g.w_bytes = (unsigned)w_bytes;
+    return FD_OK;
+}
+
+extern "C" int fd_gemm_rowres_ok(const fd_gemm_desc* d) {
+    RowresArgs g;
+    int form = 0, waves = 0;
+    return rowres_check(d, g, &form, &waves);
+}
+
+template <int FORM, int WAVES, int ST>
+static int rowres_launch(const RowresArgs& g, hipStream_t st) {
+    constexpr int lds = RR_LDS_BYTES(WAVES, ST);
+    static std::atomic<unsigned long long> configured{0};
+    if (fd_first_on_device(&configured)) {
+        FD_HIP(hipFuncSetAttribute(reinterpret_cast<const void*>(k_gemm_rowres<FORM, WAVES, ST>), hipFuncAttributeMaxDynamicSharedMemorySize, lds));
+        fd_done_on_device(&configured);
+    }
+    hipLaunchKernelGGL((k_gemm_rowres<FORM, WAVES, ST>), dim3(g.M / (WAVES * 32)), dim3(WAVES * 64), lds, st, g);
+    FD_CHECK_LAUNCH("k_gemm_rowres");
+    return FD_OK;
+}
+
+extern "C" int fd_gemm_rowres_f16(const fd_gemm_desc* d, void* stream) {
+    if (fd_plan_recording() && d) {
+        const fd_gemm_desc dc_ = *d;
+        fd_plan_push([dc_](void* fd_s_) -> int { return fd_gemm_rowres_f16(&dc_, fd_s_); });
+    }
+    RowresArgs g;
+    int form = 0, waves = 0;
+    const int rc0 = rowres_check(d, g, &form, &waves);
+    if (rc0 != FD_OK) return rc0;
+    hipStream_t st = (hipStream_t)stream;
+    const double flops = 2.0 * (double)g.M * g.N * RR_K;
+    fd_prof_begin(FD_FAMILY_GEMM, st, flops, flops, fd_tag(16u, g.M, g.N, RR_K, form * 16 + waves, g.tr_n0));
+    const int rc = waves == 8 ? (form == 0 ? rowres_launch<0, 8, 6>(g, st) : rowres_launch<1, 8, 6>(g, st))
+                              : (form == 0 ? rowres_launch<0, 4, 3>(g, st) : rowres_launch<1, 4, 3>(g, st));
+    fd_prof_end(FD_FAMILY_GEMM, st);
+    return rc;
+}
diff --git a/flexdiffuse_amd/csrc/norm.hip b/flexdiffuse_amd/csrc/norm.hip
--- a/flexdiffuse_amd/csrc/norm.hip
+++ b/flexdiffuse_amd/csrc/norm.hip
@@ -235,6 +235,7 @@
             *rc = FD_EHIP;
             return true;
         }
+        fd_done_on_device(&attr_set);
     }
     fd_prof_begin(FD_FAMILY_GROUPNORM, st, (double)B * HW * C * 4.0, -1.0, fd_tag(7u, B, HW, C, NT));
     hipLaunchKernelGGL((k_gn_slab<NT, NV>), dim3(B, G / GB), dim3(NT), lds, st, (const half_t*)x,
diff --git a/flexdiffuse_amd/csrc/xattn.hip b/flexdiffuse_amd/csrc/xattn.hip
--- a/flexdiffuse_amd/csrc/xattn.hip
+++ b/flexdiffuse_amd/csrc/xattn.hip
@@ -398,8 +398,10 @@
     typedef XaCfg<D> cfg;
     constexpr size_t lds = 2 * (size_t)(cfg::BM + 320) * 128 + (2 * 320 + 2 * cfg::BM) * sizeof(float);
     static std::atomic<unsigned long long> configured{0};
-    if (fd_first_on_device(&configured))
+    if (fd_first_on_device(&configured)) {
         FD_HIP(hipFuncSetAttribute(reinterpret_cast<const void*>(k_xattn<D>), hipFuncAttributeMaxDynamicSharedMemorySize, (int)lds));
+        fd_done_on_device(&configured);
+    }
     hipLaunchKernelGGL(k_xattn<D>, dim3(g.M / cfg::BM, n_rep, cfg::C / 320), dim3(1024), lds, st, g, a_bytes, w_bytes, o_bytes);
     return FD_OK;
 }
diff --git a/flexdiffuse_amd/hip.py b/flexdiffuse_amd/hip.py
--- a/flexdiffuse_amd/hip.py
+++ b/flexdiffuse_amd/hip.py
@@ -45,6 +45,8 @@
     'fd_gemm_plan': (c_int, [c_void_p, c_void_p, c_void_p]),
     'fd_gemm_can_fuse_groupnorm': (c_int, [c_int, c_int, c_int, c_int, c_int]),
     'fd_gemm_gn_parts_chunks': (c_int, [P]),
+    'fd_gemm_rowres_f16': (c_int, [P, P]),
+    'fd_gemm_rowres_ok': (c_int, [P]),
     'fd_groupnorm_apply_parts_f16': (c_int, [P, c_int, P, P, P, P, c_int, c_int, c_int, c_int, c_int, c_float, c_int, P]),
     'fd_groupnorm_fold_linear_parts_f16': (c_int, [P, c_int, c_int, c_int, c_int, c_int, c_float, P, P, c_int, P, P, P]),
     'fd_attention_f16': (c_int, [P, P]),
diff --git a/flexdiffuse_amd/ops.py b/flexdiffuse_amd/ops.py
--- a/flexdiffuse_amd/ops.py
+++ b/flexdiffuse_amd/ops.py
@@ -330,12 +330,27 @@
     d.ln_stats, d.ln_colsum = ln_stats.data_ptr(), w.colsum.data_ptr()
 
 
+ROWRES = int(os.environ.get('FD_GEMM_ROWRES', '1'))
+rowres_launches = 0
+
+
+def _rowres(d: 'fd_gemm_desc', asked: bool) -> bool:
+    global rowres_launches
+    if ROWRES <= 0 or (ROWRES == 1 and not asked) or d.K != 320:
+        return False
+    if hip.lib().fd_gemm_rowres_ok(ctypes.byref(d)) != hip.FD_OK:
+        return False
+    hip.call('fd_gemm_rowres_f16', ctypes.byref(d), hip.stream())
+    rowres_launches += 1
+    return True
+
+
 def gemm(a: torch.Tensor, w: LinW, *, act: int = ACT_NONE, residual: Optional[torch.Tensor] = None,
          bias2: Optional[torch.Tensor] = None, ld_bias2: int = 0, rows_per_sample: int = 0,
          out_f32: bool = False, out: Optional[torch.Tensor] = None, alpha: float = 1.0,
          use_bias: bool = True, ln_stats: Optional[torch.Tensor] = None,
          ln_stats_out: Optional[torch.Tensor] = None, ln_eps: float = 1e-5,
-         a2: Optional[torch.Tensor] = None, gn_parts: int = 0):
+         a2: Optional[torch.Tensor] = None, gn_parts: int = 0, rowres: bool = False):
     M, K = a.shape
     K2 = 0 if a2 is None else a2.shape[1]
     assert a.dtype == torch.float16 and a.stride(1) == 1 and K + K2 == w.K, (a.shape, K2, w.K)
@@ -365,6 +380,8 @@
     if ln_stats_out is not None:
         assert ln_stats_out.shape[-2:] == (M, 2) and ln_stats_out.dtype == torch.float32 and ln_stats_out.is_contiguous()
         d.ln_stats_out, d.ln_eps = ln_stats_out.data_ptr(), ln_eps
+    if act == ACT_GEGLU and ln_stats is not None and not gn_parts and _rowres(d, rowres):
+        return out
     _sched(d, a.device)
     if gn_parts:
         parts = _gn_parts_request(d, M // rows_per_sample, gn_parts, a) if rows_per_sample > 0 and M % rows_per_sample == 0 else None
@@ -405,7 +422,8 @@
     return QKV_MERGE and M % 128 == 0 and C % 160 == 0 and rows_per_sample % 32 == 0 and M % rows_per_sample == 0
 
 
-def gemm_qkv(a: torch.Tensor, w: LinW, B: int, rows_per_sample: int, ln_stats: torch.Tensor) -> Tuple[torch.Tensor, torch.Tensor]:
+def gemm_qkv(a: torch.Tensor, w: LinW, B: int, rows_per_sample: int, ln_stats: torch.Tensor,
+             rowres: bool = False) -> Tuple[torch.Tensor, torch.Tensor]:
     M, K = a.shape
     C = w.N // 3
     assert w.N == 3 * C and K == w.K and M == B * rows_per_sample and w.colsum is not None
@@ -419,7 +437,8 @@
     d.rows_per_sample, d.alpha, d.batch = rows_per_sample, 1.0, 1
     d.trans_n0, d.trans_ld, d.trans_sample_stride = 2 * C, rows_per_sample, C * rows_per_sample
     _set_ln_stats(d, ln_stats, w, M)
-    hip.call('fd_gemm_f16', ctypes.byref(d), hip.stream())
+    if not _rowres(d, rowres):
+        hip.call('fd_gemm_f16', ctypes.byref(d), hip.stream())
     return qk, vt
 
 
diff --git a/flexdiffuse_amd/unet.py b/flexdiffuse_amd/unet.py
--- a/flexdiffuse_amd/unet.py
+++ b/flexdiffuse_amd/unet.py
@@ -335,6 +335,12 @@
             return int(lo or 0) <= M <= int(hi or (1 << 30))
         return not (8192 <= M <= 16384)
 
+    ROWRES_ROWS = {'G': (), 'Q': (65536, 32768)}
+
+    @classmethod
+    def _rowres_level(cls, form: str, M: int) -> bool:
+        return M in cls.ROWRES_ROWS[form]
+
     def _gn1(self, r: Optional[_Res]) -> Optional[ops.GNSpec]:
         return None if r is None else ops.GNSpec(r.n1g, r.n1b, self.G, 1e-5, True)
 
@@ -389,7 +395,7 @@
         if a.ln_fold:
             st = fin(st, h, parts_ok=True)
             if a.qkv1 is not None and ops.qkv_merge_supported(B * HW, C, HW) and self._qkv_level(B * HW):
-                qk, vt = ops.gemm_qkv(h, a.qkv1, B, HW, st)
+                qk, vt = ops.gemm_qkv(h, a.qkv1, B, HW, st, rowres=self._rowres_level('Q', B * HW))
             else:
                 qk = ops.gemm(h, a.qk1, ln_stats=st)
                 vt = ops.gemm_vt(h, a.v1, B, HW, (HW + 7) // 8 * 8, ln_stats=st)
@@ -437,7 +443,8 @@
             st = mkst(B * HW)
             h = ops.gemm(o, a.o2, residual=h, ln_stats_out=st)
         if a.ln_fold:
-            f = ops.gemm(h, a.ff1, act=ops.ACT_GEGLU, ln_stats=fin(st, h, parts_ok=C >= 1280))
+            f = ops.gemm(h, a.ff1, act=ops.ACT_GEGLU, ln_stats=fin(st, h, parts_ok=C >= 1280),
+                         rowres=C == 320 and self._rowres_level('G', h.shape[0]))
         else:
             f = ops.gemm(ops.layernorm(h, *a.ln[2]), a.ff1, act=ops.ACT_GEGLU)
         if a.ffp is not None:
diff --git a/include/flexdiffuse_hip.h b/include/flexdiffuse_hip.h
--- a/include/flexdiffuse_hip.h
+++ b/include/flexdiffuse_hip.h
@@ -125,6 +125,8 @@
 int fd_gemm_plan(const fd_gemm_desc* d, int* tile, int* split_k);
 int fd_gemm_can_fuse_groupnorm(int M, int N, int rows_per_sample, int groups, int split_k);
 int fd_gemm_gn_parts_chunks(const fd_gemm_desc* d);
+int fd_gemm_rowres_f16(const fd_gemm_desc* desc, void* stream);
+int fd_gemm_rowres_ok(const fd_gemm_desc* desc);
 int fd_xattn_fold_rows_f32(const void* kf, const void* K, const float* bias_q, float* rows, int samples, int n_keys, int heads, int head_dim,
                            int C, int ldk, void* stream);
 
```

New measurement: 10.97 images/sec (median of 6 runs). Within noise of the previous version (+0.3%).
